# zorino/kaamer

Measured on AMD Instinct MI355X. Metric: k-mer lookups/sec, higher is better.
Workload: dtype u32

## Files before the change

kaamer_amd/csrc/count_async.hip.inc:

```

#define CA_NCTX 2u
#define CA_ARENA (GRP_BUDGET - 64u + GRP_MAX_TABLE)
#define CA_NONE 0xFFFFFFFFu
#define GRP_WQ 64u

template <bool FIRSTPOS>
__global__ __launch_bounds__(64 * GRP_WAVES, FIRSTPOS ? 5 : 6) void count_async_kernel(CountParams p)
{
    constexpr int WAVES = GRP_WAVES;
    constexpr int XIT = 2;
    constexpr bool PACKED = FIRSTPOS;
    __shared__ uint32_t a_keys[CA_ARENA];
    __shared__ uint32_t a_cnt[CA_ARENA];
    __shared__ uint32_t c_q[CA_NCTX][GRP_QMAX];
    __shared__ uint16_t c_tab[CA_NCTX][GRP_QMAX], c_cap[CA_NCTX][GRP_QMAX];
    __shared__ uint8_t c_ovf[CA_NCTX][GRP_QMAX];
    __shared__ uint32_t c_pref[CA_NCTX][GRP_QMAX + 1];
    __shared__ uint64_t c_aa[CA_NCTX][GRP_QMAX];
    __shared__ uint32_t c_hits[CA_NCTX][GRP_QMAX];
    __shared__ uint8_t c_wq[CA_NCTX][GRP_WQ];
    __shared__ uint8_t c_sq[CA_NCTX][CA_ARENA / 64];
    __shared__ uint32_t c_seq[CA_NCTX];
    __shared__ uint32_t c_nq[CA_NCTX], c_npos[CA_NCTX], c_nwin[CA_NCTX], c_tb[CA_NCTX];
    __shared__ uint32_t c_str0[CA_NCTX], c_nstr[CA_NCTX];
    __shared__ uint32_t c_need[CA_NCTX];
    __shared__ unsigned long long c_ebase[CA_NCTX];
    __shared__ uint32_t c_wdone[CA_NCTX], c_sticket[CA_NCTX], c_sdone[CA_NCTX];
    __shared__ uint32_t c_retired[CA_NCTX];
    __shared__ uint2 s_ent[CA_NCTX];
    __shared__ uint32_t s_ticket;
    __shared__ uint32_t s_built, s_tb_end, s_arena_end, s_build_lock, s_nret;
    __shared__ uint32_t s_hint;
    __shared__ uint32_t s_pref[WAVES][64];
    __shared__ uint8_t s_own[WAVES][XIT * 64];
    __shared__ unsigned long long s_tot[8];
    enum { T_IN = 0, T_Q, T_POST, T_HITS, T_OVF, T_LISTS, T_LIDS };

    const uint32_t tid = threadIdx.x, lane = tid & 63u, wv = tid >> 6;
#ifdef KAAMER_PHASE_CLOCK
    const unsigned long long ca_t0 = PHASE_T();
    unsigned long long ca_win = 0, ca_str = 0, ca_bld = 0, ca_idle = 0, ca_nwin = 0;
#define CA_CLK(acc, expr) { const unsigned long long t_ = PHASE_T(); expr; acc += PHASE_T() - t_; }
#else
#define CA_CLK(acc, expr) { expr; }
#endif
    const unsigned long long below = (1ull << lane) - 1ull;
    const uint32_t n_groups = *p.d_n_groups;
    const uint32_t nq_total = *p.d_nq;
    const uint32_t n_sched_raw = *p.d_n_sched;
    const uint32_t n_sched = n_sched_raw & 0x7FFFFFFFu;
    const bool sched_identity = (n_sched_raw >> 31) != 0u;
    const uint32_t K = n_sched > blockIdx.x ? (n_sched - 1u - blockIdx.x) / gridDim.x + 1u : 0u;
    if (K == 0u) return;

    auto ld = [&](uint32_t *w) { return __hip_atomic_load(w, __ATOMIC_RELAXED, __HIP_MEMORY_SCOPE_WORKGROUP); };
    auto st = [&](uint32_t *w, uint32_t v) { __hip_atomic_store(w, v, __ATOMIC_RELAXED, __HIP_MEMORY_SCOPE_WORKGROUP); };
    auto uni = [&](uint32_t v) { return (uint32_t)__builtin_amdgcn_readfirstlane((int)v); };
    auto sched_entry = [&](uint32_t k) {
        const uint32_t t = blockIdx.x + k * gridDim.x;
        if (k >= K) return make_uint2(0xFFFFFFFFu, GRP_NONE);
        const uint2 e = sched_identity ? make_uint2(t, p.group_first[t]) : p.sched[t];
        return make_uint2(uni(e.x), uni(e.y));
    };

    if (tid < 8) s_tot[tid] = 0;
    for (uint32_t i = tid; i < WAVES * XIT * 64; i += 64 * WAVES) (&s_own[0][0])[i] = 0;
    for (uint32_t i = tid; i < CA_ARENA; i += 64 * WAVES) {
        a_keys[i] = KH_EMPTY_PID;
        a_cnt[i] = PACKED ? 0xFFFF0000u : 0u;
    }
    if (tid == 0) {
        s_ticket = 0; s_built = 0; s_tb_end = 0; s_arena_end = 0; s_build_lock = 0; s_nret = 0; s_hint = 0;
        for (uint32_t c = 0; c < CA_NCTX; c++) { c_seq[c] = CA_NONE; c_retired[c] = 0; c_wdone[c] = 0; c_sticket[c] = 0; c_sdone[c] = 0; c_nwin[c] = 0; c_nstr[c] = 0; }
    }
    if (wv == 0) { const uint2 e = sched_entry(0u); if (lane == 0) s_ent[0] = e; }
    __syncthreads();

    auto retire = [&](uint32_t c) {
        const uint32_t nqp = c_nq[c];
        if (lane < nqp) {
            const uint32_t j = lane, q = c_q[c][j];
            if (c_ovf[c][j]) {
                atomicAdd(&s_tot[T_OVF], 1ull);
                const uint32_t slot = atomicAdd(p.ovf_count, 1u);
                WorkItem wi;
                wi.q = q; wi.size = p.qinfo[q].size; wi.aa_off = c_aa[c][j];
                if (slot < p.list_cap) p.ovf_list[slot] = wi;
                else atomicOr(p.status, (uint32_t)ST_LIST_FULL);
                p.q_cnt[q] = 0;
                p.hit_off[q] = 0;
            } else {
                const unsigned long long base = c_ebase[c] + c_tab[c][j];
                const bool have = base + c_cap[c][j] <= p.hit_cap;
                if (!have) atomicOr(p.status, (uint32_t)ST_POOL_FULL);
                p.q_cnt[q] = have ? c_hits[c][j] : 0u;
                p.hit_off[q] = have ? base : 0;
            }
        }
        __builtin_amdgcn_fence(__ATOMIC_RELEASE, "workgroup", "local");
        if (lane == 0) {
            st(&c_retired[c], ld(&c_seq[c]) + 1u);
            atomicAdd(&s_nret, 1u);
            atomicAdd(&s_hint, 1u);
        }
    };

    auto build = [&](uint32_t k) {
        const uint32_t c = k & 1u;
        if (lane == 0) st(&c_seq[c], CA_NONE);
        __builtin_amdgcn_fence(__ATOMIC_RELEASE, "workgroup", "local");
        const uint2 e = s_ent[c];
        const uint32_t gidb = e.x, firstb = e.y;
        const uint2 en = sched_entry(k + 1u);
        QInfo pre_qi;
        pre_qi.size = 0; pre_qi.slots = 0; pre_qi.aa_off = 0;
        uint64_t pre_e = 0;
        if (firstb != GRP_NONE && gidb < n_groups && (uint64_t)firstb + lane < nq_total) { pre_qi = p.qinfo[firstb + lane]; pre_e = p.slot_off[firstb + lane]; }
        const uint64_t e_first = __shfl(pre_e, 0, 64);
        uint32_t nq = 0, pos_carry = 0, slots_end = 0;
        uint64_t q0 = firstb;
        bool done = firstb == GRP_NONE || gidb >= n_groups;
        while (!done) {
            const uint64_t q = q0 + lane;
            const bool in_range = q < nq_total;
            QInfo qi;
            qi.size = 0; qi.slots = 0; qi.aa_off = 0;
            uint64_t eq = 0;
            if (q0 == firstb) { qi = pre_qi; eq = pre_e; }
            else if (in_range) { qi = p.qinfo[q]; eq = p.slot_off[q]; }
            const bool searched = in_range && qi.slots != 0;
            const bool beyond = !in_range || (searched && (eq >> GRP_SHIFT) > gidb);
            const unsigned long long bm = __ballot(beyond);
            const uint32_t cutoff = bm ? (uint32_t)__ffsll((long long)bm) - 1 : 64u;
            const bool mine = searched && lane < cutoff;
            const unsigned long long mm = __ballot(mine);
            const uint32_t szm = mine ? (uint32_t)qi.size : 0u;
            const uint32_t inc = wave_inclusive_scan_dpp(szm);
            const uint32_t tab = (uint32_t)(eq - e_first);
            if (mine) {
                const uint32_t idx = nq + (uint32_t)__popcll(mm & below);
                if (idx < GRP_QMAX) {
                    const uint32_t lo = pos_carry + inc - szm, hi = pos_carry + inc;
                    c_q[c][idx] = (uint32_t)q;
                    c_aa[c][idx] = qi.aa_off;
                    c_tab[c][idx] = (uint16_t)tab;
                    c_cap[c][idx] = (uint16_t)qi.slots;
                    c_ovf[c][idx] = (PACKED && qi.size >= 65535) ? 1u : 0u;
                    c_pref[c][idx] = lo;
                    c_hits[c][idx] = 0u;
                    for (uint32_t w = (lo + 63u) >> 6; (w << 6) < hi && w < GRP_WQ; w++) c_wq[c][w] = (uint8_t)idx;
                }
            }
            if (mm) {
                const int last = 63 - __builtin_clzll(mm);
                slots_end = (uint32_t)__builtin_amdgcn_readlane((int)(tab + qi.slots), last);
            }
            pos_carry += (uint32_t)__builtin_amdgcn_readlane((int)inc, 63);
            nq += (uint32_t)__popcll(mm);
            done = bm != 0;
            q0 += 64;
        }
        if (nq > GRP_QMAX) nq = GRP_QMAX;
        if (slots_end > CA_ARENA) slots_end = CA_ARENA;
        const uint32_t prev_end = ld(&s_arena_end);
        const uint32_t base = prev_end + slots_end <= CA_ARENA ? prev_end : 0u;
        uint32_t need = CA_NONE;
        if (k > 0u) {
            const uint32_t pc = c ^ 1u;
            const uint32_t pb = ld(&c_str0[pc]) << 6, pe = pb + (ld(&c_nstr[pc]) << 6);
            if (base < pe && pb < base + slots_end) need = k - 1u;
        }
        __builtin_amdgcn_fence(__ATOMIC_ACQ_REL, "wavefront");
        __builtin_amdgcn_wave_barrier();
        if (lane < nq) {
            const uint32_t t0 = base + c_tab[c][lane], cp = c_cap[c][lane];
            c_tab[c][lane] = (uint16_t)t0;
            for (uint32_t s = t0 >> 6; s < ((t0 + cp) >> 6) && s < CA_ARENA / 64; s++) c_sq[c][s] = (uint8_t)lane;
        }
        const uint32_t n_win = (pos_carry + 63u) >> 6;
        __builtin_amdgcn_fence(__ATOMIC_RELEASE, "workgroup", "local");
        if (lane == 0) {
            c_pref[c][nq] = pos_carry;
            c_nq[c] = nq; c_npos[c] = pos_carry; c_nwin[c] = n_win;
            c_str0[c] = base >> 6; c_nstr[c] = slots_end >> 6;
            c_need[c] = need;
            c_ebase[c] = e_first - (unsigned long long)base;
            const uint32_t tb = ld(&s_tb_end);
            c_tb[c] = tb;
            st(&s_tb_end, tb + n_win);
            st(&s_arena_end, base + slots_end);
            c_wdone[c] = 0; c_sticket[c] = 0; c_sdone[c] = 0;
            s_ent[c ^ 1u] = en;
            atomicAdd(&s_tot[T_Q], (unsigned long long)nq);
            atomicAdd(&s_tot[T_IN], (unsigned long long)pos_carry + 6ull * nq);
        }
        __builtin_amdgcn_fence(__ATOMIC_RELEASE, "workgroup", "local");
        if (lane == 0) st(&c_seq[c], k);
        if (n_win == 0u) {
            retire(c);
        }
        __builtin_amdgcn_fence(__ATOMIC_RELEASE, "workgroup", "local");
        if (lane == 0) { st(&s_built, k + 1u); st(&s_build_lock, 0u); }
    };
    auto try_build = [&]() -> bool {
        const uint32_t k = ld(&s_built);
        if (k >= K) return false;
        if (k >= CA_NCTX && ld(&c_retired[k & 1u]) != k - 1u) return false;
        uint32_t got = 0;
        if (lane == 0) got = atomicCAS(&s_build_lock, 0u, 1u) == 0u ? 1u : 0u;
        if (!uni(got)) return false;
        __builtin_amdgcn_fence(__ATOMIC_ACQUIRE, "workgroup", "local");
        if (ld(&s_built) != k) { if (lane == 0) st(&s_build_lock, 0u); return false; }
        build(k);
        return true;
    };

    auto try_stripes = [&](uint32_t c) -> bool {
        const uint32_t sq = uni(ld(&c_seq[c]));
        if (sq == CA_NONE) return false;
        const uint32_t nw = uni(ld(&c_nwin[c])), nst = uni(ld(&c_nstr[c]));
        const uint32_t wd = uni(ld(&c_wdone[c])), stk = uni(ld(&c_sticket[c]));
        __builtin_amdgcn_fence(__ATOMIC_ACQUIRE, "workgroup", "local");
        if (uni(ld(&c_seq[c])) != sq) return false;
        if (nw == 0u || wd != nw || stk >= nst) return false;
        bool did = false;
        const uint32_t s0 = uni(ld(&c_str0[c]));
        const unsigned long long ebase = c_ebase[c];
        constexpr uint32_t CA_SCH = 4;
        for (;;) {
            uint32_t t = 0;
            if (lane == 0) t = atomicAdd(&c_sticket[c], CA_SCH);
            t = uni(t);
            if (t >= nst) break;
            did = true;
            const uint32_t n_here = nst - t < CA_SCH ? nst - t : CA_SCH;
            uint32_t kk[CA_SCH], ww[CA_SCH], jj[CA_SCH];
#pragma unroll
            for (uint32_t u = 0; u < CA_SCH; u++) {
                const uint32_t s = s0 + t + (u < n_here ? u : 0u);
                const uint32_t slot = (s << 6) + lane;
                jj[u] = (uint32_t)c_sq[c][s];
                kk[u] = a_keys[slot];
                ww[u] = a_cnt[slot];
            }
            uint32_t tb_[CA_SCH], cp_[CA_SCH], ov_[CA_SCH];
#pragma unroll
            for (uint32_t u = 0; u < CA_SCH; u++) {
                jj[u] = uni(jj[u]);
                tb_[u] = c_tab[c][jj[u]]; cp_[u] = c_cap[c][jj[u]]; ov_[u] = c_ovf[c][jj[u]];
            }
#pragma unroll
            for (uint32_t u = 0; u < CA_SCH; u++) {
                if (u >= n_here) break;
                const uint32_t slot = ((s0 + t + u) << 6) + lane;
                a_keys[slot] = KH_EMPTY_PID;
                a_cnt[slot] = PACKED ? 0xFFFF0000u : 0u;
                const unsigned long long base = ebase + tb_[u];
                const bool usable = ov_[u] == 0u && base + cp_[u] <= p.hit_cap;
                const bool has = usable && kk[u] != KH_EMPTY_PID;
                const unsigned long long bm = __ballot(has);
                if (bm) {
                    uint32_t off = 0;
                    if (lane == 0) {
                        off = atomicAdd(&c_hits[c][jj[u]], (uint32_t)__popcll(bm));
                        atomicAdd(&s_tot[T_HITS], (unsigned long long)__popcll(bm));
                    }
                    off = uni(off);
                    if (has) {
                        const unsigned long long idx = base + off + (uint32_t)__popcll(bm & below);
                        p.hit_pid[idx] = kk[u];
                        p.hit_km[idx] = PACKED ? (ww[u] & 0xFFFFu) : ww[u];
                        if (FIRSTPOS) p.hit_fp[idx] = ww[u] >> 16;
                    }
                }
            }
            __builtin_amdgcn_fence(__ATOMIC_RELEASE, "workgroup", "local");
            uint32_t d = 0;
            if (lane == 0) d = atomicAdd(&c_sdone[c], n_here);
            if (uni(d) + n_here == nst) { __builtin_amdgcn_fence(__ATOMIC_ACQUIRE, "workgroup", "local"); retire(c); break; }
        }
        return did;
    };
    auto help = [&]() -> bool {
        bool did = false, d2 = false;
        CA_CLK(ca_str, did = try_stripes(0u); did = try_stripes(1u) || did);
        CA_CLK(ca_bld, d2 = try_build());
        return did || d2;
    };

    struct Job { uint32_t valid, w, c, npos, nq, need; };
    uint32_t my_k = 0;
    bool at_end = false;
    uint32_t g_tb = 0, g_nw = 0, g_c = 0, g_npos = 0, g_nq = 0, g_need = CA_NONE;
    auto try_resolve = [&](uint32_t t, Job &j) -> bool {
        for (;;) {
            if (t - g_tb < g_nw) { j.valid = 1u; j.w = t - g_tb; j.c = g_c; j.npos = g_npos; j.nq = g_nq; j.need = g_need; return true; }
            if (my_k >= K) { at_end = true; j.valid = 0u; j.w = 0u; j.c = 0u; j.npos = 0u; j.nq = 0u; j.need = CA_NONE; return true; }
            if (uni(ld(&s_built)) <= my_k) return false;
            __builtin_amdgcn_fence(__ATOMIC_ACQUIRE, "workgroup", "local");
            const uint32_t c = my_k & 1u;
            if (uni(ld(&c_seq[c])) == my_k) {
                const uint32_t tb = ld(&c_tb[c]), nw = ld(&c_nwin[c]), np = ld(&c_npos[c]), nqq = ld(&c_nq[c]), nd = ld(&c_need[c]);
                __builtin_amdgcn_fence(__ATOMIC_ACQUIRE, "workgroup", "local");
                if (uni(ld(&c_seq[c])) != my_k) continue;
                if (t - uni(tb) < uni(nw)) {
                    g_tb = uni(tb); g_nw = uni(nw); g_c = c; g_npos = uni(np); g_nq = uni(nqq); g_need = uni(nd);
                    continue;
                }
            }
            g_nw = 0u;
            my_k++;
        }
    };
    struct RawA { uint32_t vraw, j, ps; };
    auto issue_a = [&](const Job &jb) {
        RawA r;
        const uint32_t c = jb.c, w = jb.w;
        const uint32_t nqb = jb.nq, npb = jb.npos;
        const uint32_t i = (w << 6) + lane;
        const bool valid = jb.valid != 0u && i < npb;
        uint32_t j = 0;
        if (valid) {
            if (w < GRP_WQ) {
                j = c_wq[c][w];
                while (j + 1 < nqb && c_pref[c][j + 1] <= i) j++;
            } else {
#pragma unroll
                for (uint32_t sft = GRP_QMAX / 2; sft > 0; sft >>= 1)
                    if (j + sft < nqb && c_pref[c][j + sft] <= i) j += sft;
            }
        }
        r.j = j;
        r.ps = valid ? i - c_pref[c][j] : 0u;
        r.vraw = p.vals[valid ? c_aa[c][j] + r.ps : 0ull];
        return r;
    };
    auto lane_valid = [&](const Job &jb) { return jb.valid != 0u && ((jb.w << 6) + lane) < jb.npos; };
    auto issue_b = [&](uint32_t v) { return reinterpret_cast<const uint4 *>(p.arena)[(v & KH_INLINE_BIT) ? 0u : v]; };

    uint32_t c_post = 0, c_lists = 0, c_lids = 0;
    uint32_t *const pref = s_pref[wv];
    uint8_t *const own = s_own[wv];
    auto add_n = [&](uint32_t c, uint32_t j, uint32_t pid, uint32_t pos, uint32_t n) {
        const uint32_t base = c_tab[c][j], cap = c_cap[c][j];
        uint32_t hh = (uint32_t)(((uint64_t)(pid * 0x9E3779B1u) * cap) >> 32);
        const uint32_t tmax = cap < GRP_MAX_PROBES ? cap : GRP_MAX_PROBES;
        for (uint32_t t = 0; t < tmax; t++) {
            const uint32_t old = atomicCAS(&a_keys[base + hh], KH_EMPTY_PID, pid);
            const uint32_t kk = old == KH_EMPTY_PID ? pid : old;
            if (kk == pid) {
                atomicAdd(&a_cnt[base + hh], n);
                if (PACKED) {
                    uint32_t o = __hip_atomic_load(&a_cnt[base + hh], __ATOMIC_RELAXED, __HIP_MEMORY_SCOPE_WORKGROUP);
                    while (pos < (o >> 16)) {
                        const uint32_t seen = atomicCAS(&a_cnt[base + hh], o, (o & 0xFFFFu) | (pos << 16));
                        if (seen == o) break;
                        o = seen;
                    }
                }
                return;
            }
            hh = (hh + 1u == cap) ? 0u : hh + 1u;
        }
        c_ovf[c][j] = 1;
    };
    auto add_runs = [&](uint32_t c, uint32_t j, uint32_t x, uint32_t pos) {
        const uint32_t px = __shfl_up(x, 1, 64), pj = __shfl_up(j, 1, 64);
        const bool change = (lane == 0) || px != x || pj != j;
        const unsigned long long cm = __ballot(change);
        if (change && x != KH_EMPTY_PID) {
            const unsigned long long above = (lane == 63) ? 0ull : (cm >> (lane + 1));
            const uint32_t len = above ? (uint32_t)__ffsll((long long)above) : 64u - lane;
            add_n(c, j, x, pos, len);
        }
    };
    auto count_window = [&](uint32_t c, uint32_t v, uint32_t wj, uint32_t wps, const uint4 &hv) {
        const uint32_t inl = (v & KH_INLINE_BIT) ? 0xFFFFFFFFu : 0u;
        const uint32_t lcnt = hv.x | (inl & 1u), id0 = hv.y | (inl & v & ~KH_INLINE_BIT);
        if (lcnt > c_cap[c][wj] && lcnt != 0u) c_ovf[c][wj] = 1u;
        const bool dead = lcnt != 0u && c_ovf[c][wj] != 0u;
        if (lcnt != 0u) {
            c_post += lcnt;
            if (!(v & KH_INLINE_BIT)) { c_lists++; c_lids += lcnt; }
        }
        const uint32_t extra = (lcnt > 1u && !dead) ? lcnt - 1u : 0u;
        const uint32_t inc = wave_inclusive_scan_dpp(extra);
        const uint32_t xtotal = (uint32_t)__builtin_amdgcn_readlane((int)inc, 63);
        pref[lane] = inc - extra;
        if (extra != 0u && inc - extra < XIT * 64u) own[inc - extra] = (uint8_t)(lane + 1u);
        __builtin_amdgcn_fence(__ATOMIC_ACQ_REL, "wavefront");
        __builtin_amdgcn_wave_barrier();
        uint32_t carry = 0;
        uint32_t xid[XIT], xld[XIT], xm[XIT], xj[XIT], xps[XIT];
#pragma unroll
        for (int it = 0; it < XIT; it++) {
            const uint32_t t = (uint32_t)it * 64u + lane;
            const bool act = t < xtotal;
            uint32_t mk = own[t];
            own[t] = 0;
            mk = wave_inclusive_max_dpp(mk > carry ? mk : carry);
            carry = (uint32_t)__builtin_amdgcn_readlane((int)mk, 63);
            const uint32_t lo = act ? mk - 1u : 0u;
            const uint32_t off = __shfl(v, (int)lo, 64);
            const uint32_t oz = __shfl(hv.z, (int)lo, 64), ow = __shfl(hv.w, (int)lo, 64);
            xj[it] = __shfl(wj, (int)lo, 64);
            xps[it] = __shfl(wps, (int)lo, 64);
            const uint32_t k = act ? t - pref[lo] : 0u;
            const bool from_arena = act && k >= 2u;
            xld[it] = p.arena[from_arena ? (uint64_t)off * 4 + 2 + k : 0ull];
            xm[it] = from_arena ? 0xFFFFFFFFu : 0u;
            xid[it] = !act ? KH_EMPTY_PID : k == 0u ? oz : ow;
        }
        add_runs(c, wj, (lcnt > 0 && !dead) ? id0 : KH_EMPTY_PID, wps);
#pragma unroll
        for (int it = 0; it < XIT; it++) {
            const uint32_t id = (xld[it] & xm[it]) | (xid[it] & ~xm[it]);
            if (id != KH_EMPTY_PID) add_n(c, xj[it], id, xps[it], 1u);
        }
        if (xtotal > XIT * 64u) {
            for (uint32_t t0 = XIT * 64u; t0 < xtotal; t0 += GRP_LONG_UNROLL * 64u) {
                uint32_t lid[GRP_LONG_UNROLL], lj[GRP_LONG_UNROLL], lp[GRP_LONG_UNROLL];
#pragma unroll
                for (int u = 0; u < (int)GRP_LONG_UNROLL; u++) {
                    const uint32_t t = t0 + (uint32_t)u * 64u + lane;
                    const bool act = t < xtotal;
                    const uint32_t tt = act ? t : xtotal - 1u;
                    uint32_t lo = 0;
#pragma unroll
                    for (int sft = 32; sft > 0; sft >>= 1)
                        if (pref[lo + sft] <= tt) lo += sft;
                    const uint32_t off = __shfl(v, (int)lo, 64);
                    const uint32_t oz = __shfl(hv.z, (int)lo, 64), ow = __shfl(hv.w, (int)lo, 64);
                    lj[u] = __shfl(wj, (int)lo, 64);
                    lp[u] = __shfl(wps, (int)lo, 64);
                    const uint32_t k = tt - pref[lo];
                    const uint32_t ldv = p.arena[k >= 2u ? (uint64_t)off * 4 + 2 + k : 0ull];
                    const uint32_t m = k >= 2u ? 0xFFFFFFFFu : 0u;
                    const uint32_t idr = k == 0u ? oz : ow;
                    lid[u] = act ? ((ldv & m) | (idr & ~m)) : KH_EMPTY_PID;
                }
#pragma unroll
                for (int u = 0; u < (int)GRP_LONG_UNROLL; u++)
                    if (lid[u] != KH_EMPTY_PID && !c_ovf[c][lj[u]]) add_n(c, lj[u], lid[u], lp[u], 1u);
            }
        }
        __builtin_amdgcn_fence(__ATOMIC_ACQ_REL, "wavefront");
        __builtin_amdgcn_wave_barrier();
    };

    if (wv == 0) build(0u);
    __syncthreads();
    if (wv == 1 && K > 1u) {
        uint32_t got = 0;
        if (lane == 0) got = atomicCAS(&s_build_lock, 0u, 1u) == 0u ? 1u : 0u;
        if (uni(got)) build(1u);
    }

    Job j0, j1;
    j0.valid = j1.valid = 0u; j0.w = j1.w = 0u; j0.c = j1.c = 0u; j0.npos = j1.npos = 0u; j0.nq = j1.nq = 0u; j0.need = j1.need = CA_NONE;
    RawA a0, a1;
    a0.vraw = a0.j = a0.ps = 0u;
    a1 = a0;
    uint32_t v0 = 0;
    uint4 hv0 = make_uint4(0, 0, 0, 0);
    uint32_t tp = 0;
    bool have_tp = false;
    uint32_t spins = 0, seen_hint = 0xFFFFFFFFu;
    for (;;) {
        Job j2;
        j2.valid = 0u; j2.w = 0u; j2.c = 0u; j2.npos = 0u; j2.nq = 0u; j2.need = CA_NONE;
        if (!at_end) {
            if (!have_tp) {
                if (lane == 0) tp = atomicAdd(&s_ticket, 1u);
                tp = uni(tp);
                have_tp = true;
            }
            if (try_resolve(tp, j2)) have_tp = false;
            else if (!j0.valid && !j1.valid) {
                if (!help()) { CA_CLK(ca_idle, __builtin_amdgcn_s_sleep(2)); if (++spins > (1u << 24)) { if (lane == 0) atomicOr(p.status, (uint32_t)ST_CHAIN_TIMEOUT); break; } }
                continue;
            }
        }
        if (at_end && !j0.valid && !j1.valid && !j2.valid) break;
        const RawA a2 = issue_a(j2);
        const uint32_t v1 = lane_valid(j1) ? a1.vraw : 0u;
        const uint4 hv1 = issue_b(v1);
        if (j0.valid) {
            const uint32_t c = j0.c;
            const uint32_t need = j0.need;
            if (need != CA_NONE) {
                while (ld(&c_retired[need & 1u]) <= need) {
                    if (!help()) { CA_CLK(ca_idle, __builtin_amdgcn_s_sleep(1)); if (++spins > (1u << 24)) { if (lane == 0) atomicOr(p.status, (uint32_t)ST_CHAIN_TIMEOUT); break; } }
                }
                __builtin_amdgcn_fence(__ATOMIC_ACQUIRE, "workgroup", "local");
            }
            CA_CLK(ca_win, count_window(c, v0, a0.j, a0.ps, hv0));
#ifdef KAAMER_PHASE_CLOCK
            ca_nwin++;
#endif
            __builtin_amdgcn_fence(__ATOMIC_RELEASE, "workgroup", "local");
            if (lane == 0 && atomicAdd(&c_wdone[c], 1u) + 1u == (j0.npos + 63u) >> 6) atomicAdd(&s_hint, 1u);
        }
        a0 = a1; v0 = v1; hv0 = hv1; a1 = a2;
        j0 = j1; j1 = j2;
        {
            const uint32_t h = uni(ld(&s_hint));
            if (h != seen_hint) { seen_hint = h; help(); }
        }
    }
    while (ld(&s_nret) < K) {
        if (!help()) { CA_CLK(ca_idle, __builtin_amdgcn_s_sleep(2)); if (++spins > (1u << 24)) { if (lane == 0) atomicOr(p.status, (uint32_t)ST_CHAIN_TIMEOUT); break; } }
    }
    {
        const uint32_t a = wave_total(c_post), b = wave_total(c_lists), c = wave_total(c_lids);
        if (lane == 0) {
            atomicAdd(&s_tot[T_POST], (unsigned long long)a);
            atomicAdd(&s_tot[T_LISTS], (unsigned long long)b);
            atomicAdd(&s_tot[T_LIDS], (unsigned long long)c);
        }
    }
#ifdef KAAMER_PHASE_CLOCK
    if (lane == 0 && blockIdx.x < 2048) {
        unsigned long long *g = g_phase_clock[blockIdx.x];
        atomicAdd(&g[0], ca_nwin); atomicAdd(&g[1], ca_win); atomicAdd(&g[2], ca_str); atomicAdd(&g[3], ca_bld); atomicAdd(&g[4], ca_idle);
        atomicAdd(&g[5], PHASE_T() - ca_t0); atomicAdd(&g[7], 1ull);
    }
#endif
    __syncthreads();
    if (tid == 0) {
        const uint32_t rep = blockIdx.x;
        add_counter(p.counters, rep, CTR_IN, s_tot[T_IN]);
        add_counter(p.counters, rep, CTR_QUERIES, s_tot[T_Q]);
        add_counter(p.counters, rep, CTR_POST, s_tot[T_POST]);
        add_counter(p.counters, rep, CTR_HITS, s_tot[T_HITS]);
        add_counter(p.counters, rep, CTR_OVERFLOW, s_tot[T_OVF]);
        add_counter(p.counters, rep, CTR_LISTS, s_tot[T_LISTS]);
        add_counter(p.counters, rep, CTR_LIST_IDS, s_tot[T_LIDS]);
    }
}
#undef CA_CLK
```

kaamer_amd/csrc/count_group.hip.inc:

```

#ifndef GRP_WAVES
#define GRP_WAVES 8
#endif
#ifndef GRP_BUDGET
#define GRP_BUDGET 2048u
#endif
#define GRP_SHIFT 11u
static_assert((1u << GRP_SHIFT) == GRP_BUDGET, "GRP_BUDGET must be 1 << GRP_SHIFT");
#define GRP_MAX_TABLE 4096u
#define GRP_MIN_TABLE 64u
#define GRP_ARENA (GRP_BUDGET + GRP_MAX_TABLE)
#define GRP_QMAX (GRP_BUDGET / GRP_MIN_TABLE)
#define GRP_FIT (GRP_BUDGET - 64u + GRP_MAX_TABLE)
#define GRP_NONE 0xFFFFFFFFu
#define GRP_MAX_PROBES 96u
#ifndef GRP_NWIN
#define GRP_NWIN 1
#endif
#ifndef GRP_V2
#define GRP_V2 1
#endif
#ifndef GRP_LONG_UNROLL
#define GRP_LONG_UNROLL 4u
#endif
// ... 46 lines not shown
    __shared__ uint64_t s_w[LAY_THREADS / 64];
    __shared__ uint64_t s_prefix;
    const uint32_t nq = *d_nq;
    const uint64_t base = (uint64_t)blockIdx.x * LAY_TILE;
    if (base > nq) return;
    const uint32_t tid = threadIdx.x, lane = tid & 63u, wv = tid >> 6;
    uint32_t v[LAY_ITEMS];
    uint64_t sum = 0;
    const uint64_t i0 = base + (uint64_t)tid * LAY_ITEMS;
#pragma unroll
    for (int i = 0; i < LAY_ITEMS; i++) {
        v[i] = i0 + i < nq ? slots[i0 + i] : 0u;
        sum += v[i];
    }
    uint64_t inc = sum;
#pragma unroll
    for (int o = 1; o < 64; o <<= 1) {
        const uint64_t t = __shfl_up(inc, o, 64);
        if ((int)lane >= o) inc += t;
    }
    if (lane == 63) s_w[wv] = inc;
    __syncthreads();
    uint64_t woff = 0, tile_total = 0;
#pragma unroll
    for (int i = 0; i < LAY_THREADS / 64; i++) {
        if (i < (int)wv) woff += s_w[i];
        tile_total += s_w[i];
    }
    if (wv == 0) {
        unsigned long long prefix = 0;
        if (blockIdx.x > 0) {
            if (lane == 0)
                __hip_atomic_store(&chain[blockIdx.x], chain_pack(epoch, 1u, tile_total), __ATOMIC_RELAXED, __HIP_MEMORY_SCOPE_AGENT);
            long long j = (long long)blockIdx.x - 1;
            uint32_t spins = 0;
            bool done = false;
            while (!done) {
                const long long idx = j - (long long)lane;
                unsigned long long w = chain_pack(epoch, 2u, 0ull);
                if (idx >= 0) w = __hip_atomic_load(&chain[idx], __ATOMIC_RELAXED, __HIP_MEMORY_SCOPE_AGENT);
                const uint32_t flag = (uint32_t)(w >> (CHAIN_VAL_BITS + 2)) == epoch ? (uint32_t)(w >> CHAIN_VAL_BITS) & 3u : 0u;
                const unsigned long long m_inc = __ballot(flag == 2u), m_inv = __ballot(flag == 0u);
                const uint32_t first_inc = m_inc ? (uint32_t)__ffsll((long long)m_inc) - 1u : 64u;
                const unsigned long long need = first_inc >= 63u ? ~0ull : ((2ull << first_inc) - 1ull);
                if (m_inv & need) {
                    if (++spins > (1u << 20)) { if (lane == 0) atomicOr(status, (uint32_t)ST_CHAIN_TIMEOUT); break; }
                    __builtin_amdgcn_s_sleep(1);
                    continue;
                }
                unsigned long long part = lane <= first_inc ? (w & CHAIN_VAL_MASK) : 0ull;
#pragma unroll
                for (int o = 32; o > 0; o >>= 1) part += __shfl_xor(part, o, 64);
                prefix += part;
                done = first_inc < 64u;
                j -= 64;
            }
        }
        if (lane == 0) {
            __hip_atomic_store(&chain[blockIdx.x], chain_pack(epoch, 2u, prefix + tile_total), __ATOMIC_RELAXED, __HIP_MEMORY_SCOPE_AGENT);
            s_prefix = prefix;
        }
    }
    __syncthreads();
    uint64_t ex = s_prefix + woff + inc - sum;
    if (i0 == 0 && nq > 0 && groups_cap > 0) { group_first[0] = 0u; group_start[0] = 0; }
#pragma unroll
    for (int i = 0; i < LAY_ITEMS; i++) {
        const uint64_t idx = i0 + i;
        if (idx <= nq) E[idx] = ex;
        if (idx == nq) {
            uint64_t ng = ex ? ((ex - 1) >> bshift) + 1 : 0;
            if (ng > groups_cap) { atomicOr(status, (uint32_t)ST_LIST_FULL); ng = 0; }
            *d_n_groups = (uint32_t)ng;
        }
        if (idx < nq && v[i]) {
            const uint64_t g = ex >> bshift, g_hi = (ex + v[i]) >> bshift;
            for (uint64_t gg = g + 1; gg <= g_hi && gg < groups_cap; gg++) {
                group_first[gg] = gg == g_hi ? (uint32_t)(idx + 1) : GRP_NONE;
                group_start[gg] = ex + v[i];
            }
        }
        ex += v[i];
    }
}

#define SCHED_MAX_GROUPS 32768u
__global__ __launch_bounds__(1024) void schedule_kernel(const uint32_t *group_first, const uint64_t *group_start, const uint64_t *E,
                                                        const uint32_t *d_n_groups, const uint32_t *d_nq, uint2 *sched, uint32_t *d_n_sched,
                                                        uint32_t cshift)
{
    __shared__ uint32_t s_hist[16], s_base[16], s_cur[16];
    __shared__ uint8_t s_cls[SCHED_MAX_GROUPS];
    const uint32_t ng = *d_n_groups, tid = threadIdx.x;
    if (ng > SCHED_MAX_GROUPS) {
        if (tid == 0) *d_n_sched = ng | 0x80000000u;
        return;
    }
    const uint64_t total = E[*d_nq];
    if (tid < 16) { s_hist[tid] = 0; s_cur[tid] = 0; }
    __syncthreads();
    for (uint32_t g = tid; g < ng; g += 1024) {
        uint32_t c = 0xFFu;
        if (group_first[g] != GRP_NONE) {
            const uint64_t ext = (g + 1 < ng ? group_start[g + 1] : total) - group_start[g];
            c = (uint32_t)(ext >> cshift);
            c = c > 15u ? 15u : c;
            atomicAdd(&s_hist[c], 1u);
        }
        s_cls[g] = (uint8_t)c;
    }
    __syncthreads();
    if (tid == 0) {
        uint32_t run = 0;
        for (int c = 15; c >= 0; c--) { s_base[c] = run; run += s_hist[c]; }
        *d_n_sched = run;
    }
    __syncthreads();
    for (uint32_t g = tid; g < ng; g += 1024) {
        const uint32_t c = s_cls[g];
        if (c != 0xFFu) sched[s_base[c] + atomicAdd(&s_cur[c], 1u)] = make_uint2(g, group_first[g]);
    }
}

struct PrepLayoutParams {
    const uint8_t *seqs;
    const uint64_t *offsets;
    uint32_t n_seqs;
    uint64_t pos_bound;
    kaamer_query_meta *q;
    uint32_t *d_nq;
    unsigned long long *d_n_pos;
    unsigned long long *invalid;
    QInfo *qinfo;
    uint64_t *hit_off;
    uint32_t *q_cnt;
    uint64_t *E;
    uint32_t *group_first;
    uint64_t *group_start;
    uint32_t *d_n_groups;
    uint32_t groups_cap;
    unsigned long long *chain;
    uint32_t epoch;
    uint32_t *status;
    uint2 *sched;
    uint32_t *d_n_sched;
    uint32_t *slots;
    uint32_t bshift;
    uint32_t cshift;
    uint32_t no_sched;
    uint32_t *tiles_done;
    unsigned long long *d_total;
    const uint32_t *slot_scale;
    unsigned long long room_slots;
};

#define PL_ITEMS 1
#define PL_TILE (LAY_THREADS * PL_ITEMS)
__global__ __launch_bounds__(LAY_THREADS) void prep_layout_schedule_kernel(PrepLayoutParams p)
{
    __shared__ uint64_t s_w[LAY_THREADS / 64];
    __shared__ uint64_t s_prefix;
    __shared__ uint32_t s_slots[PL_TILE];
    __shared__ uint32_t s_last;
    const uint32_t nq = p.n_seqs;
    const uint64_t base = (uint64_t)blockIdx.x * PL_TILE;
    const uint32_t tid = threadIdx.x, lane = tid & 63u, wv = tid >> 6;
    const bool batch_bad = p.offsets[nq] > p.pos_bound;
    const uint32_t slot_scale = p.slot_scale ? fit_table_scale(*p.slot_scale, batch_bad ? 0ull : p.offsets[nq], nq, p.room_slots) : SLOT_SCALE_ONE;
    if (blockIdx.x == 0 && tid == 0) {
        const uint64_t n_pos = batch_bad ? 0 : p.offsets[nq];
        if (batch_bad) atomicOr(p.status, (uint32_t)ST_AA_CAP);
        *p.d_nq = nq;
        *p.d_n_pos = n_pos;
        mark_invalid_range(p.invalid, n_pos, (n_pos + 63) & ~63ull);
    }
#pragma unroll
    for (int r = 0; r < PL_ITEMS; r++) {
        const uint64_t i = base + (uint64_t)r * LAY_THREADS + tid;
        uint32_t slots = 0;
        if (i < nq) {
            uint64_t b = p.offsets[i], e = p.offsets[i + 1];
            if (batch_bad || e < b || e > p.pos_bound) {
                if (!batch_bad) atomicOr(p.status, (uint32_t)ST_AA_CAP);
                b = e = 0;
            }
            const int64_t len = (int64_t)(e - b);
            int32_t size = (int32_t)(len - KAAMER_KMER_SIZE + 1);
            if (len > 0 && p.seqs[e - 1] == '*') size--;
            kaamer_query_meta m;
            m.src_seq = (uint32_t)i;
            m.size_in_kmer = size;
            m.start_position = 1;
            m.end_position = (int32_t)len;
            m.plus_strand = 1;
            m.aa_len = (uint32_t)len;
            m.aa_off = b;
            m.sa_off = 0;
            m.sa_len = 0;
            p.q[i] = m;
            p.q_cnt[i] = 0;
            p.hit_off[i] = 0;
            QInfo qi;
            qi.size = size;
            qi.aa_off = b;
            if (size >= 7) {
                qi.slots = table_slots_for(size, slot_scale);
                mark_invalid_range(p.invalid, b + (uint64_t)size, e);
            } else {
                qi.slots = 0;
                mark_invalid_range(p.invalid, b, e);
            }
            p.qinfo[i] = qi;
            p.slots[i] = qi.slots;
            slots = qi.slots;
        }
        s_slots[r * LAY_THREADS + tid] = slots;
    }
    __syncthreads();
    uint32_t v[PL_ITEMS];
    uint64_t sum = 0;
    const uint64_t i0 = base + (uint64_t)tid * PL_ITEMS;
#pragma unroll
    for (int i = 0; i < PL_ITEMS; i++) {
        v[i] = s_slots[tid * PL_ITEMS + i];
        sum += v[i];
    }
    uint64_t inc = sum;
#pragma unroll
    for (int o = 1; o < 64; o <<= 1) {
        const uint64_t t = __shfl_up(inc, o, 64);
        if ((int)lane >= o) inc += t;
    }
    if (lane == 63) s_w[wv] = inc;
    __syncthreads();
    uint64_t woff = 0, tile_total = 0;
#pragma unroll
    for (int i = 0; i < LAY_THREADS / 64; i++) {
        if (i < (int)wv) woff += s_w[i];
        tile_total += s_w[i];
    }
    if (wv == 0) {
        unsigned long long prefix = 0;
        if (blockIdx.x > 0) {
            if (lane == 0)
                __hip_atomic_store(&p.chain[blockIdx.x], chain_pack(p.epoch, 1u, tile_total), __ATOMIC_RELAXED, __HIP_MEMORY_SCOPE_AGENT);
            long long j = (long long)blockIdx.x - 1;
            uint32_t spins = 0;
            bool done = false;
            while (!done) {
                const long long idx = j - (long long)lane;
                unsigned long long w = chain_pack(p.epoch, 2u, 0ull);
                if (idx >= 0) w = __hip_atomic_load(&p.chain[idx], __ATOMIC_RELAXED, __HIP_MEMORY_SCOPE_AGENT);
                const uint32_t flag = (uint32_t)(w >> (CHAIN_VAL_BITS + 2)) == p.epoch ? (uint32_t)(w >> CHAIN_VAL_BITS) & 3u : 0u;
                const unsigned long long m_inc = __ballot(flag == 2u), m_inv = __ballot(flag == 0u);
                const uint32_t first_inc = m_inc ? (uint32_t)__ffsll((long long)m_inc) - 1u : 64u;
                const unsigned long long need = first_inc >= 63u ? ~0ull : ((2ull << first_inc) - 1ull);
                if (m_inv & need) {
                    if (++spins > (1u << 20)) { if (lane == 0) atomicOr(p.status, (uint32_t)ST_CHAIN_TIMEOUT); break; }
                    __builtin_amdgcn_s_sleep(1);
                    continue;
                }
                unsigned long long part = lane <= first_inc ? (w & CHAIN_VAL_MASK) : 0ull;
#pragma unroll
                for (int o = 32; o > 0; o >>= 1) part += __shfl_xor(part, o, 64);
                prefix += part;
                done = first_inc < 64u;
                j -= 64;
            }
        }
        if (lane == 0) {
            __hip_atomic_store(&p.chain[blockIdx.x], chain_pack(p.epoch, 2u, prefix + tile_total), __ATOMIC_RELAXED, __HIP_MEMORY_SCOPE_AGENT);
            s_prefix = prefix;
        }
    }
    __syncthreads();
    uint64_t ex = s_prefix + woff + inc - sum;
    if (i0 == 0 && nq > 0 && p.groups_cap > 0) {
        __hip_atomic_store(&p.group_first[0], 0u, __ATOMIC_RELAXED, __HIP_MEMORY_SCOPE_AGENT);
        __hip_atomic_store(&p.group_start[0], (uint64_t)0, __ATOMIC_RELAXED, __HIP_MEMORY_SCOPE_AGENT);
    }
#pragma unroll
    for (int i = 0; i < PL_ITEMS; i++) {
        const uint64_t idx = i0 + i;
        if (idx <= nq) p.E[idx] = ex;
        if (idx == nq) {
            uint64_t ng = ex ? ((ex - 1) >> p.bshift) + 1 : 0;
            if (ng > p.groups_cap) { atomicOr(p.status, (uint32_t)ST_LIST_FULL); ng = 0; }
            __hip_atomic_store(p.d_n_groups, (uint32_t)ng, __ATOMIC_RELAXED, __HIP_MEMORY_SCOPE_AGENT);
            __hip_atomic_store(p.d_total, (unsigned long long)ex, __ATOMIC_RELAXED, __HIP_MEMORY_SCOPE_AGENT);
            if (p.no_sched) *p.d_n_sched = (uint32_t)ng | 0x80000000u;
        }
        if (idx < nq && v[i]) {
            const uint64_t g = ex >> p.bshift, g_hi = (ex + v[i]) >> p.bshift;
            for (uint64_t gg = g + 1; gg <= g_hi && gg < p.groups_cap; gg++) {
                __hip_atomic_store(&p.group_first[gg], gg == g_hi ? (uint32_t)(idx + 1) : GRP_NONE, __ATOMIC_RELAXED, __HIP_MEMORY_SCOPE_AGENT);
                __hip_atomic_store(&p.group_start[gg], (uint64_t)(ex + v[i]), __ATOMIC_RELAXED, __HIP_MEMORY_SCOPE_AGENT);
            }
        }
        ex += v[i];
    }
    if (p.no_sched) return;
    asm volatile("s_waitcnt vmcnt(0) lgkmcnt(0)" ::: "memory");
    __syncthreads();
    if (tid == 0) s_last = atomicAdd(p.tiles_done, 1u) == gridDim.x - 1u;
    __syncthreads();
    if (!s_last) return;
    if (tid == 0) __hip_atomic_store(p.tiles_done, 0u, __ATOMIC_RELAXED, __HIP_MEMORY_SCOPE_AGENT);
    uint32_t *s_hist = s_slots, *s_base = s_slots + 16, *s_cur = s_slots + 32;
    __shared__ uint8_t s_cls[SCHED_MAX_GROUPS];
    const uint32_t ng = __hip_atomic_load(p.d_n_groups, __ATOMIC_RELAXED, __HIP_MEMORY_SCOPE_AGENT);
    if (ng > SCHED_MAX_GROUPS) {
        if (tid == 0) *p.d_n_sched = ng | 0x80000000u;
        return;
    }
    const uint64_t total = __hip_atomic_load(p.d_total, __ATOMIC_RELAXED, __HIP_MEMORY_SCOPE_AGENT);
    if (tid < 16) { s_hist[tid] = 0; s_cur[tid] = 0; }
    __syncthreads();
    for (uint32_t g = tid; g < ng; g += LAY_THREADS) {
        uint32_t c = 0xFFu;
        if (__hip_atomic_load(&p.group_first[g], __ATOMIC_RELAXED, __HIP_MEMORY_SCOPE_AGENT) != GRP_NONE) {
            const uint64_t nxt = g + 1 < ng ? __hip_atomic_load(&p.group_start[g + 1], __ATOMIC_RELAXED, __HIP_MEMORY_SCOPE_AGENT) : total;
            const uint64_t ext = nxt - __hip_atomic_load(&p.group_start[g], __ATOMIC_RELAXED, __HIP_MEMORY_SCOPE_AGENT);
            c = (uint32_t)(ext >> p.cshift);
            c = c > 15u ? 15u : c;
            atomicAdd(&s_hist[c], 1u);
        }
        s_cls[g] = (uint8_t)c;
    }
    __syncthreads();
    if (tid == 0) {
        uint32_t run = 0;
        for (int c = 15; c >= 0; c--) { s_base[c] = run; run += s_hist[c]; }
        *p.d_n_sched = run;
    }
    __syncthreads();
    for (uint32_t g = tid; g < ng; g += LAY_THREADS) {
        const uint32_t c = s_cls[g];
        if (c != 0xFFu)
            p.sched[s_base[c] + atomicAdd(&s_cur[c], 1u)] =
                make_uint2(g, __hip_atomic_load(&p.group_first[g], __ATOMIC_RELAXED, __HIP_MEMORY_SCOPE_AGENT));
    }
}

__device__ __forceinline__ uint32_t wave_inclusive_scan_dpp(uint32_t v)
{
#define KH_DPP_ADD(ctrl, rmask) v += (uint32_t)__builtin_amdgcn_update_dpp(0, (int)v, ctrl, rmask, 0xf, false)
    KH_DPP_ADD(0x111, 0xf);
    KH_DPP_ADD(0x112, 0xf);
    KH_DPP_ADD(0x114, 0xf);
    KH_DPP_ADD(0x118, 0xf);
    KH_DPP_ADD(0x142, 0xa);
    KH_DPP_ADD(0x143, 0xc);
#undef KH_DPP_ADD
    return v;
}

__device__ __forceinline__ uint32_t wave_inclusive_max_dpp(uint32_t v)
{
#define KH_DPP_MAX(ctrl, rmask) { const uint32_t t_ = (uint32_t)__builtin_amdgcn_update_dpp(0, (int)v, ctrl, rmask, 0xf, false); v = v > t_ ? v : t_; }
    KH_DPP_MAX(0x111, 0xf);
    KH_DPP_MAX(0x112, 0xf);
    KH_DPP_MAX(0x114, 0xf);
    KH_DPP_MAX(0x118, 0xf);
// ... 820 lines not shown
```

kaamer_amd/csrc/search.hip:

```cpp
#include <hip/hip_runtime.h>

#include <dlfcn.h>

#include <algorithm>
#include <cstdarg>
#include <cstdio>
#include <cstdlib>
#include <cstring>
#include <condition_variable>
#include <memory>
#include <mutex>
#include <new>
#include <vector>

#include "kaamer_internal.h"

static thread_local char g_err[512] = "";

int kaamer_fail(int code, const char *fmt, ...)
{
    va_list ap;
    va_start(ap, fmt);
    vsnprintf(g_err, sizeof g_err, fmt, ap);
    va_end(ap);
    return code;
}

#define HIPCHK(expr)                                                                          \
    do {                                                                                      \
        hipError_t e_ = (expr);                                                               \
        if (e_ != hipSuccess)                                                                 \
            return kaamer_fail(KAAMER_E_HIP, "%s failed: %s", #expr, hipGetErrorString(e_)); \
    } while (0)

struct kaamer_workspace;
struct HostSlot {
    kaamer_workspace *ws = nullptr;
    kaamer_workspace_opts opts{};
    uint8_t *d_seqs = nullptr;
    uint64_t *d_off = nullptr;
    size_t seq_cap = 0, off_cap = 0;
    hipStream_t stream = nullptr;
    bool busy = false;
};

struct TopSlot {
    kaamer_workspace *ws = nullptr;
    kaamer_workspace_opts opts{};
    hipStream_t stream = nullptr;
    uint8_t *d_seqs = nullptr;
    uint64_t *d_off = nullptr;
    size_t seq_cap = 0, off_cap = 0;
    uint8_t *h_in = nullptr;
    size_t h_in_cap = 0;
    uint8_t *d_block = nullptr;
    size_t d_block_cap = 0;
    size_t guess = 1u << 16;
    bool busy = false;
};
#define KAAMER_MAX_HOST_SLOTS 8
static void top_slot_free(TopSlot &h);

struct kaamer_index {
    int device;
    kh_image_header hdr;
    kh_bucket *d_buckets;
    uint32_t *d_arena;
    HostSlot host[4];
    std::mutex pool_mu;
    std::condition_variable pool_cv;
    TopSlot top[KAAMER_MAX_HOST_SLOTS];
    int n_top;
};

enum { ST_POOL_FULL = 1u, ST_LIST_FULL = 2u, ST_QUERY_CAP = 4u, ST_AA_CAP = 8u, ST_G_ARENA_FULL = 16u, ST_G_TABLE_FULL = 32u,
       ST_POS_UNSUPPORTED = 64u, ST_POS_CAP = 128u, ST_CHAIN_TIMEOUT = 256u, ST_EXCHANGE_CAP = 512u, ST_PEER_FAILED = 1024u };
enum { CTR_IN = 0, CTR_QUERIES, CTR_LOOKUP, CTR_PROBE, CTR_FOUND, CTR_POST, CTR_HITS, CTR_OVERFLOW, CTR_LISTS, CTR_LIST_IDS, CTR_N };
static_assert(sizeof(kaamer_counters) == CTR_N * 8, "counter layout");
#define CTR_REPLICAS 64

enum { LIST_S = 0, LIST_L, LIST_SO, LIST_G, N_LISTS };
enum { SLOT_QUEUE_HEAD = N_LISTS, SLOT_STATUS = N_LISTS + 1, SLOT_GROUP_QUEUE = N_LISTS + 2, SLOT_GROUP_QUEUE_POS = N_LISTS + 3,
       SLOT_N_LONG = N_LISTS + 4, SLOT_TILES_DONE = N_LISTS + 5, SLOT_TR_TICKET = N_LISTS + 6,
       SLOT_QUEUE_SUB = N_LISTS + 7 , SLOT_G_TICKET = N_LISTS + 15, SLOT_PACK_TICKETS = N_LISTS + 16 ,
       SLOT_G_HITS16 = N_LISTS + 80 ,
       SLOT_G_MON_HITS16 = N_LISTS + 81 , SLOT_G_MONSTERS = N_LISTS + 82 ,
       N_SMALL_SLOTS = N_LISTS + 16 + 64 + 3 };
#define G_MONSTER_HITS (GRP_MAX_TABLE / 4u * 3u)
static_assert(N_SMALL_SLOTS <= 256, "the finalize step zeroes one slot per thread");
struct alignas(16) WorkItem {
    uint32_t q;
    int32_t size;
    uint64_t aa_off;
};

#define CURSOR_STRIDE 32u
#define MAX_TIMED_CALLS 1024u
#define L_WAVES 8
#define L_LOG2CAP 12
#define G_WAVES 8
#ifndef S_MIN_WAVES
#define S_MIN_WAVES 1
#endif
#ifndef L_MIN_WAVES
#define L_MIN_WAVES 1
#endif
#ifndef S_NWIN
#define S_NWIN 3
#endif

__device__ __forceinline__ uint32_t lane_id() { return threadIdx.x & 63u; }

__device__ __forceinline__ uint32_t wave_sum32(uint32_t v)
{
#pragma unroll
    for (int o = 32; o > 0; o >>= 1) v += __shfl_xor(v, o, 64);
    return v;
}
__device__ __forceinline__ uint32_t wave_total(uint32_t v)
{
    return (uint32_t)__builtin_amdgcn_readfirstlane((int)wave_sum32(v));
}

__device__ __forceinline__ void add_counter(unsigned long long *replicas, uint32_t replica, int which, unsigned long long v)
{
    if (v) atomicAdd(&replicas[(size_t)(replica % CTR_REPLICAS) * CTR_N + which], v);
}

struct ProbeParams {
    const uint4 *table;
    uint64_t n_buckets;
    uint32_t n_shards, shard;
    const uint8_t *residues;
    unsigned long long *invalid;
    const unsigned long long *d_n_pos;
    uint32_t *vals;
    unsigned long long *counters;
    uint32_t nontemporal;
};

#define P_WAVES 4
#define P_RING 128u
#define KH_NO_KEY 0xFFFFFFFDu

template <bool SKIP_IDLE> __global__ __launch_bounds__(64 * P_WAVES) void probe_kernel(ProbeParams p)
{
    __shared__ uint8_t s_lut[256];
    __shared__ uint8_t s_stage[P_WAVES][80];
    __shared__ uint32_t s_ring[P_WAVES][3][P_RING];
    const uint32_t tid = threadIdx.x, lane = tid & 63u;
    const uint32_t wv = (uint32_t)__builtin_amdgcn_readfirstlane((int)(tid >> 6));
    const unsigned long long n_pos = *p.d_n_pos;
    const unsigned long long n_win = (n_pos + 63) >> 6;
    for (uint32_t i = tid; i < 256; i += 64 * P_WAVES) s_lut[i] = (uint8_t)kh_residue_code((uint8_t)i);
    __syncthreads();
    uint32_t c_lookup = 0, c_probe = 0, c_found = 0;
    uint8_t *stage = s_stage[wv];
    uint32_t *const ring_key = s_ring[wv][0], *const ring_pos = s_ring[wv][1], *const ring_step = s_ring[wv][2];
    uint32_t ring_head = 0, ring_n = 0;
    const uint32_t n_buckets = (uint32_t)p.n_buckets;
    const uint32_t mine = 16u * (lane & 3u) + (lane >> 2);

    const unsigned long long stride = (unsigned long long)gridDim.x * P_WAVES;
    unsigned long long w = (unsigned long long)blockIdx.x * P_WAVES + wv;
    unsigned long long mask = 0;
    uint32_t ra = 0, rb = 0;
    auto fetch = [&](unsigned long long win, unsigned long long &m, uint32_t &a, uint32_t &b) {
        const unsigned long long wc = win < n_win ? win : n_win - 1;
        m = p.invalid[wc];
        const unsigned long long i0 = (wc << 6) + lane, last = n_pos - 1;
        a = p.residues[i0 < last ? i0 : last];
        b = p.residues[i0 + 64 < last ? i0 + 64 : last];
    };
    if (n_win) fetch(w, mask, ra, rb);

    while (n_win) {
        const bool ring = ring_n >= 64u || (w >= n_win && ring_n > 0u);
        if (!ring && w >= n_win) break;
        unsigned long long base = 0;
        uint32_t key = KH_NO_KEY, off = lane, step = 0;
        if (ring) {
            const uint32_t n = ring_n < 64u ? ring_n : 64u;
            if (lane < n) {
                const uint32_t slot = (ring_head + lane) & (P_RING - 1u);
                key = ring_key[slot]; off = ring_pos[slot]; step = ring_step[slot];
            }
            ring_head = (ring_head + n) & (P_RING - 1u);
            ring_n -= n;
        } else {
            base = w << 6;
            stage[lane] = s_lut[ra];
            if (lane < 6) stage[64 + lane] = s_lut[rb];
            __builtin_amdgcn_fence(__ATOMIC_ACQ_REL, "wavefront");
            __builtin_amdgcn_wave_barrier();
            const uint8_t *st = stage + lane;
            key = kh_key_from_codes(st[0], st[1], st[2], st[3], st[4], st[5], st[6]);
            const bool own = p.n_shards <= 1 || kh_shard_of(key, p.n_shards) == p.shard;
            key = (((~mask >> lane) & 1ull) && own) ? key : KH_NO_KEY;
            __builtin_amdgcn_fence(__ATOMIC_ACQ_REL, "wavefront");
            __builtin_amdgcn_wave_barrier();
            c_lookup += key != KH_NO_KEY ? 1u : 0u;
        }
        c_probe += key != KH_NO_KEY ? 1u : 0u;
        const unsigned long long w_cur = w;
        if (!ring) w += stride;
        fetch(w, mask, ra, rb);

        uint32_t my_bucket = 0u;
        if (key != KH_NO_KEY) {
            my_bucket = (uint32_t)kh_home_bucket(key, p.n_shards, p.n_buckets) + step;
            my_bucket = my_bucket >= n_buckets ? my_bucket - n_buckets : my_bucket;
        }
        uint4 ld[4];
        uint32_t rk[4];
#pragma unroll
        for (int j = 0; j < 4; j++) {
            const int src = 16 * j + (int)(lane >> 2);
            rk[j] = __shfl(key, src, 64);
            const uint32_t bucket = __shfl(my_bucket, src, 64);
            typedef uint32_t v4u __attribute__((ext_vector_type(4)));
            const v4u *srcp = reinterpret_cast<const v4u *>(p.table) + (uint64_t)bucket * 4 + (lane & 3u);
            if (SKIP_IDLE) {
                ld[j] = make_uint4(KH_EMPTY_KEY, 0u, KH_EMPTY_KEY, 0u);
                if (rk[j] != KH_NO_KEY) {
                    const v4u t = *srcp;
                    ld[j] = make_uint4(t.x, t.y, t.z, t.w);
                }
            } else {
                const v4u t = p.nontemporal ? __builtin_nontemporal_load(srcp) : *srcp;
                ld[j] = make_uint4(t.x, t.y, t.z, t.w);
            }
        }
        uint32_t okey = KH_NO_KEY, oval = 0, oempty = 1u;
#pragma unroll
        for (int j = 0; j < 4; j++) {
            const uint32_t kk = rk[j];
            uint32_t r = (ld[j].x == kk) ? ld[j].y : ((ld[j].z == kk) ? ld[j].w : 0u);
            uint32_t e = (ld[j].x == KH_EMPTY_KEY || ld[j].z == KH_EMPTY_KEY) ? 1u : 0u;
            r |= (uint32_t)__builtin_amdgcn_update_dpp(0, (int)r, 0xB1, 0xf, 0xf, false);
            e |= (uint32_t)__builtin_amdgcn_update_dpp(0, (int)e, 0xB1, 0xf, 0xf, false);
            r |= (uint32_t)__builtin_amdgcn_update_dpp(0, (int)r, 0x4E, 0xf, 0xf, false);
            e |= (uint32_t)__builtin_amdgcn_update_dpp(0, (int)e, 0x4E, 0xf, 0xf, false);
            const bool take = (lane & 3u) == (uint32_t)j;
            okey = take ? kk : okey; oval = take ? r : oval; oempty = take ? e : oempty;
        }
        const uint32_t ooff = __shfl(off, (int)mine, 64);
        const bool valid = okey != KH_NO_KEY;
        c_found += (valid && oval != 0u) ? 1u : 0u;
        const unsigned long long W = __ballot(valid && oval == 0u && oempty == 0u);
        if (W) {
            const uint32_t ostep = __shfl(step, (int)mine, 64);
            const bool wk = valid && oval == 0u && oempty == 0u && ostep + 1u < n_buckets;
            const unsigned long long W2 = __ballot(wk);
            if (wk) {
                const uint32_t slot = (ring_head + ring_n + (uint32_t)__builtin_amdgcn_mbcnt_hi((uint32_t)(W2 >> 32), __builtin_amdgcn_mbcnt_lo((uint32_t)W2, 0u))) & (P_RING - 1u);
                ring_key[slot] = okey;
                ring_pos[slot] = (uint32_t)base + ooff;
                ring_step[slot] = ostep + 1u;
            }
            ring_n += (uint32_t)__popcll(W2);
        }
        __builtin_amdgcn_fence(__ATOMIC_ACQ_REL, "wavefront");
        __builtin_amdgcn_wave_barrier();
        if (!ring || oval != 0u) p.vals[base + ooff] = oval;
        if (lane == 0) p.invalid[ring ? n_win + 1 : w_cur] = 0ull;
    }
    const uint32_t t_lookup = wave_total(c_lookup), t_probe = wave_total(c_probe), t_found = wave_total(c_found);
    if (lane == 0) {
        const uint32_t rep = blockIdx.x * P_WAVES + wv;
        add_counter(p.counters, rep, CTR_LOOKUP, t_lookup);
        add_counter(p.counters, rep, CTR_PROBE, t_probe);
        add_counter(p.counters, rep, CTR_FOUND, t_found);
    }
}

struct QInfo;
struct CountParams {
    const uint32_t *arena;
    const uint32_t *vals;
    const struct QInfo *qinfo;
    const uint64_t *slot_off;
    uint32_t *group_first;
    const uint32_t *d_n_groups;
    const uint32_t *d_nq;
    uint32_t last_group_pass;
    uint32_t pack_shift;
    uint32_t *pack_tickets;
    const uint64_t *pos_base;
    unsigned long long *pos_bits;
    const uint32_t *m_pid, *m_km, *m_fp;
    uint32_t merge_fp;
    const WorkItem *list;
    const uint32_t *list_count;
    WorkItem *ovf_list;
    uint32_t *ovf_count;
    uint32_t list_cap;
    uint32_t *queue_head;
    uint32_t *group_queue;
    const uint2 *sched;
    const uint32_t *d_n_sched;
    uint64_t *hit_off;
    uint32_t *q_cnt;
    uint32_t *hit_pid, *hit_km, *hit_fp;
    uint64_t hit_cap;
    unsigned long long *tail_cursor;
    uint32_t *g_keys;
    uint64_t g_slots;
    unsigned long long *g_cursor;
    uint32_t n_proteins;
    unsigned long long *counters;
    uint32_t *status;
    kaamer_counters *fin_out;
    uint32_t *fin_small, *fin_status_out;
    unsigned long long *fin_cursors;
    uint32_t *fin_slot_scale;
    uint32_t fin_scale_cap, fin_scale_margin;
};

__device__ __forceinline__ unsigned long long tail_alloc(const CountParams &p, uint32_t total)
{
    const unsigned long long b = p.slot_off[*p.d_nq] + atomicAdd(p.tail_cursor, (unsigned long long)total);
    if (b + total > p.hit_cap) { atomicOr(p.status, (uint32_t)ST_POOL_FULL); return ~0ull; }
    return b;
}

template <int LOG2CAP, bool FIRSTPOS = true> struct LdsTable {
    volatile uint32_t *keys;
    uint32_t *cnt, *minpos, *nd;
    static constexpr uint32_t CAP = 1u << LOG2CAP;
    static constexpr uint32_t LIMIT = CAP - CAP / 4;
    __device__ __forceinline__ bool add_n(uint32_t pid, uint32_t pos, uint32_t n, uint32_t &nnew) const
    {
        constexpr uint32_t MASK = CAP - 1u;
        uint32_t h = (pid * 0x9E3779B1u) >> (32 - LOG2CAP);
        for (uint32_t t = 0; t <= MASK; t++) {
            uint32_t k = keys[h];
            if (k == KH_EMPTY_PID) {
                const uint32_t old = atomicCAS((uint32_t *)&keys[h], KH_EMPTY_PID, pid);
                if (old == KH_EMPTY_PID) { nnew++; k = pid; }
                else k = old;
            }
            if (k == pid) {
                atomicAdd(&cnt[h], n);
                if (FIRSTPOS) atomicMin(&minpos[h], pos);
                return true;
            }
            h = (h + 1u) & MASK;
        }
        return false;
    }
    __device__ __forceinline__ bool over_limit() const { return *(volatile uint32_t *)nd > LIMIT; }
};

#define BIG_LOG2CAP 13
struct BigLdsTable {
    uint32_t *keys, *val, *nd;
    static constexpr uint32_t CAP = 1u << BIG_LOG2CAP;
    static constexpr uint32_t LIMIT = CAP - CAP / 4;
    __device__ __forceinline__ bool add_n(uint32_t pid, uint32_t pos, uint32_t n, uint32_t &nnew) const
    {
        uint32_t h = (pid * 0x9E3779B1u) >> (32 - BIG_LOG2CAP);
        for (uint32_t t = 0; t < 128u; t++) {
            uint32_t k = __hip_atomic_load(&keys[h], __ATOMIC_RELAXED, __HIP_MEMORY_SCOPE_WORKGROUP);
            if (k == KH_EMPTY_PID) {
                const uint32_t old = atomicCAS(&keys[h], KH_EMPTY_PID, pid);
                if (old == KH_EMPTY_PID) { k = pid; if (atomicAdd(nd, 1u) >= LIMIT) return false; }
                else k = old;
            }
            if (k == pid) {
                atomicAdd(&val[h], n);
                uint32_t old = __hip_atomic_load(&val[h], __ATOMIC_RELAXED, __HIP_MEMORY_SCOPE_WORKGROUP);
                while (pos < (old >> 16)) {
                    const uint32_t seen = atomicCAS(&val[h], old, (old & 0xFFFFu) | (pos << 16));
                    if (seen == old) break;
                    old = seen;
                }
                return true;
            }
            h = (h + 1u) & (CAP - 1u);
        }
        return false;
    }
    __device__ __forceinline__ bool over_limit() const { return false; }
};

#define G_MAX_RANGES 64u
__device__ __forceinline__ uint32_t g_range_of(uint32_t pid, uint32_t R) { return (uint32_t)(((uint64_t)(pid * 0x85EBCA6Bu) * R) >> 32); }
struct RangeHist {
    uint32_t *cnt, *nd;
    uint32_t R;
    __device__ __forceinline__ bool add_n(uint32_t pid, uint32_t, uint32_t, uint32_t &) const { atomicAdd(&cnt[g_range_of(pid, R)], 1u); return true; }
    __device__ __forceinline__ bool over_limit() const { return false; }
};
struct RangeScatter {
    uint32_t *cur, *nd;
    uint2 *items;
    uint32_t R;
    const uint32_t *first;
    uint32_t cap;
    uint32_t *ovf;
    __device__ __forceinline__ bool add_n(uint32_t pid, uint32_t pos, uint32_t n, uint32_t &) const
    {
        const uint32_t r = g_range_of(pid, R);
        const uint32_t at = atomicAdd(&cur[r], 1u);
        if (at - first[r] < cap) items[at] = make_uint2(pid, pos | (n << 16));
        else *ovf = 1u;
        return true;
    }
    __device__ __forceinline__ bool over_limit() const { return false; }
};

struct GlobalTable {
    uint32_t *slots;
    uint32_t *nd;
    uint32_t log2cap;
    __device__ __forceinline__ bool add_n(uint32_t pid, uint32_t pos, uint32_t n, uint32_t &nnew) const
    {
        const uint32_t mask = (1u << log2cap) - 1u;
        uint32_t h = (pid * 0x9E3779B1u) >> (32 - log2cap);
        for (uint32_t t = 0; t <= mask; t++) {
            uint32_t *sl = slots + 4ull * h;
            uint32_t k = KH_EMPTY_PID;
            if (__hip_atomic_compare_exchange_strong(&sl[0], &k, pid, __ATOMIC_RELAXED, __ATOMIC_RELAXED, __HIP_MEMORY_SCOPE_WORKGROUP)) {
                nnew++;
                k = pid;
            }
            if (k == pid) {
                __hip_atomic_fetch_add(&sl[1], n, __ATOMIC_RELAXED, __HIP_MEMORY_SCOPE_WORKGROUP);
                __hip_atomic_fetch_min(&sl[2], pos, __ATOMIC_RELAXED, __HIP_MEMORY_SCOPE_WORKGROUP);
                return true;
            }
            h = (h + 1u) & mask;
// ... 85 lines not shown
#pragma unroll
        for (int k = 0; k < NWIN; k++) {
            const volatile uint32_t *pref = s_pref + k * 64;
#pragma unroll
            for (int it = 0; it < XIT; it++) {
                const uint32_t t = (uint32_t)it * 64u + lane;
                const bool act = t < xtotal[k];
                uint32_t lo = 0;
                if (act) {
#pragma unroll
                    for (int sft = 32; sft > 0; sft >>= 1)
                        if (pref[lo + sft] <= t) lo += sft;
                }
                const uint32_t off = __shfl(v[k], (int)lo, 64);
                xid[k][it] = KH_EMPTY_PID;
                xpos[k][it] = (uint32_t)(c0 + k * stride) + lo;
                if (act) xid[k][it] = p.arena[(uint64_t)off * 4 + 4 + (t - pref[lo])];
            }
        }
#pragma unroll
        for (int k = 0; k < NWIN; k++) {
            const volatile uint32_t *pref = s_pref + k * 64;
            for (uint32_t t0 = XIT * 64u; t0 < xtotal[k]; t0 += 64) {
                const uint32_t t = t0 + lane;
                const bool act = t < xtotal[k];
                uint32_t lo = 0;
                if (act) {
#pragma unroll
                    for (int sft = 32; sft > 0; sft >>= 1)
                        if (pref[lo + sft] <= t) lo += sft;
                }
                const uint32_t off = __shfl(v[k], (int)lo, 64);
                if (act) ok = ok && tab.add_n(p.arena[(uint64_t)off * 4 + 4 + (t - pref[lo])], (uint32_t)(c0 + k * stride) + lo, 1u, nnew);
            }
        }
        __builtin_amdgcn_fence(__ATOMIC_ACQUIRE, "wavefront");
        __builtin_amdgcn_wave_barrier();
    }
#pragma unroll
    for (int k = 0; k < NWIN; k++) {
        const uint32_t pos = (uint32_t)(c0 + k * stride) + lane;
        const uint32_t lcnt = h[k].x;
        if (lcnt != 0u) {
            c.post += lcnt;
            if (!(v[k] & KH_INLINE_BIT)) { c.lists++; c.lids += lcnt; }
        }
        if (!COUNT_ONLY) {
            ok = add_runs(tab, lcnt > 0 ? h[k].y : KH_EMPTY_PID, pos, nnew) && ok;
            ok = add_runs(tab, lcnt > 1 ? h[k].z : KH_EMPTY_PID, pos, nnew) && ok;
            ok = add_runs(tab, lcnt > 2 ? h[k].w : KH_EMPTY_PID, pos, nnew) && ok;
        }
    }
    if (!COUNT_ONLY) {
#pragma unroll
        for (int k = 0; k < NWIN; k++)
#pragma unroll
            for (int it = 0; it < XIT; it++)
                if (xid[k][it] != KH_EMPTY_PID) ok = ok && tab.add_n(xid[k][it], xpos[k][it], 1u, nnew);
        const uint32_t wave_new = wave_total(nnew);
        if (lane == 0 && wave_new) atomicAdd(tab.nd, wave_new);
    }
    return __all(ok);
}

__device__ __forceinline__ void mark_invalid_range(unsigned long long *invalid, uint64_t b, uint64_t e)
{
    while (b < e) {
        const uint64_t w = b >> 6;
        const uint64_t hi = ((w + 1) << 6) < e ? ((w + 1) << 6) : e;
        const unsigned nb = (unsigned)(hi - b);
        const unsigned long long m = (nb == 64 ? ~0ull : ((1ull << nb) - 1ull)) << (b & 63);
        atomicOr(&invalid[w], m);
        b = hi;
    }
}

#include "count_group.hip.inc"
#include "count_async.hip.inc"
#define PK_ARENA_PROT 1600u
#ifndef PK_ARENA_ORF
#define PK_ARENA_ORF 640u
#endif
#define PK_ARENA_ORF_LONG 1024u
#include "count_pack.hip.inc"

struct NullTable {
    uint32_t *nd;
    __device__ __forceinline__ bool add_n(uint32_t, uint32_t, uint32_t, uint32_t &) const { return true; }
    __device__ __forceinline__ bool over_limit() const { return false; }
};

template <bool IN_FLIGHT>
__device__ __forceinline__ void finalize_body(unsigned long long *replicas, kaamer_counters *out, uint32_t *small_state,
                                              uint32_t *status_out, unsigned long long *cursors, uint32_t *slot_scale = nullptr,
                                              uint32_t scale_cap = 16u, uint32_t margin_q4 = 30u)
{
    static_assert(CTR_REPLICAS == 64, "one replica per lane");
    const uint32_t lane = threadIdx.x & 63u, wv = threadIdx.x >> 6;
    for (uint32_t c = wv; c < CTR_N; c += blockDim.x >> 6) {
        unsigned long long *w = &replicas[(size_t)lane * CTR_N + c];
        unsigned long long s = IN_FLIGHT ? __hip_atomic_load(w, __ATOMIC_RELAXED, __HIP_MEMORY_SCOPE_AGENT) : *w;
        *w = 0;
#pragma unroll
        for (int o = 32; o > 0; o >>= 1) s += __shfl_xor(s, o, 64);
        if (lane == 0) ((unsigned long long *)out)[c] = s;
    }
    unsigned long long g_hits = 0, g_mon_hits = 0, g_monsters = 0;
    if (threadIdx.x == 0) {
        *status_out = IN_FLIGHT ? __hip_atomic_load(&small_state[SLOT_STATUS], __ATOMIC_RELAXED, __HIP_MEMORY_SCOPE_AGENT) : small_state[SLOT_STATUS];
        g_hits = 16ull * (IN_FLIGHT ? __hip_atomic_load(&small_state[SLOT_G_HITS16], __ATOMIC_RELAXED, __HIP_MEMORY_SCOPE_AGENT) : small_state[SLOT_G_HITS16]);
        g_mon_hits = 16ull * (IN_FLIGHT ? __hip_atomic_load(&small_state[SLOT_G_MON_HITS16], __ATOMIC_RELAXED, __HIP_MEMORY_SCOPE_AGENT) : small_state[SLOT_G_MON_HITS16]);
        g_monsters = IN_FLIGHT ? __hip_atomic_load(&small_state[SLOT_G_MONSTERS], __ATOMIC_RELAXED, __HIP_MEMORY_SCOPE_AGENT) : small_state[SLOT_G_MONSTERS];
    }
    __syncthreads();
    if (threadIdx.x < N_SMALL_SLOTS) small_state[threadIdx.x] = 0;
    if (threadIdx.x < 3) cursors[threadIdx.x * CURSOR_STRIDE] = 0;
    if (slot_scale && threadIdx.x == 0) {
        const unsigned long long nq = out->n_queries;
        const unsigned long long n_ovf = out->n_overflow < nq ? out->n_overflow : nq;
        const unsigned long long n_mon = g_monsters < n_ovf ? g_monsters : n_ovf;
        const bool widen = 8ull * (n_ovf - n_mon) > nq;
        const unsigned long long ovf = widen ? n_mon : n_ovf;
        const unsigned long long left_out = widen ? g_mon_hits : g_hits;
        const unsigned long long hits = out->n_hits > left_out ? out->n_hits - left_out : 0ull;
        const unsigned long long lookups = nq ? out->n_lookup / nq * (nq - ovf) + out->n_lookup % nq * (nq - ovf) / nq : 0ull;
        if (lookups) {
            unsigned long long t = (hits * margin_q4 + lookups - 1ull) / lookups;
            if (t < 24ull) t = 16ull;
            if (t > scale_cap) t = scale_cap;
            *slot_scale = (uint32_t)t;
        }
    }
}

#ifndef G_MIN_BLOCKS
#define G_MIN_BLOCKS 1
#endif
#ifndef G_NWIN
#define G_NWIN 2
#endif
#ifdef KAAMER_PHASE_CLOCK
__device__ unsigned long long g_gtier_clock[2048][16];
#endif
__global__ __launch_bounds__(64 * G_WAVES, G_MIN_BLOCKS) void count_global_kernel(CountParams p)
{
    constexpr int WAVES = G_WAVES;
    __shared__ uint32_t s_nd, s_fail, s_cursor;
    constexpr int NWIN = G_NWIN;
    __shared__ uint32_t s_pref[WAVES][NWIN * 64];
    __shared__ unsigned long long s_post, s_off, s_base, s_reserved;
    __shared__ uint32_t s_roff[G_MAX_RANGES], s_rcur[G_MAX_RANGES], s_rtotal;
    __shared__ LongSink s_long;
    __shared__ uint32_t b_keys[BigLdsTable::CAP], b_val[BigLdsTable::CAP];

    const uint32_t tid = threadIdx.x, lane = tid & 63u, wv = tid >> 6;
    const uint32_t n_items = *p.list_count < p.list_cap ? *p.list_count : p.list_cap;
    const uint32_t n_part = n_items < gridDim.x ? (n_items ? n_items : 1u) : gridDim.x;
    if (blockIdx.x >= n_part) return;
    unsigned long long tot_hits = 0, f_post = 0, f_lists = 0, f_lids = 0, mon_hits = 0;
    uint32_t mon_q = 0;
#ifdef KAAMER_PHASE_CLOCK
    unsigned long long gq_acc[10] = {0, 0, 0, 0, 0, 0, 0, 0, 0, 0};
    const unsigned long long gq_start = wall_clock64();
#endif
    PostCtr pc;
    NullTable nt;
    nt.nd = &s_nd;
    auto expand_long = [&](const auto &tab) {
        const uint32_t nl = s_long.n < LONG_SINK_CAP ? s_long.n : LONG_SINK_CAP;
        if (wv == 0 && nl) {
            constexpr uint32_t PER = LONG_SINK_CAP / 64;
            uint32_t sum = 0;
            for (uint32_t i = 0; i < PER; i++) { const uint32_t e = lane * PER + i; sum += e < nl ? s_long.cnt[e] : 0u; }
            uint32_t inc = sum;
#pragma unroll
            for (int o = 1; o < 64; o <<= 1) {
                const uint32_t t = __shfl_up(inc, o, 64);
                if ((int)lane >= o) inc += t;
            }
            uint32_t run = inc - sum;
            for (uint32_t i = 0; i < PER; i++) {
                const uint32_t e = lane * PER + i;
                if (e < nl) { const uint32_t c = s_long.cnt[e]; s_long.cnt[e] = run; run += c; }
            }
            if (lane == 63) s_long.total = inc;
        }
        __syncthreads();
        uint32_t nnew = 0;
        bool ok = true;
        const uint32_t total = nl ? s_long.total : 0u;
#ifndef G_EXPAND_UNROLL
#define G_EXPAND_UNROLL 8
#endif
        constexpr int EU = G_EXPAND_UNROLL;
        uint32_t e = 0;
        auto find_list = [&](uint32_t t) {
            if (e + 1u < nl && s_long.cnt[e + 1u] <= t) {
                e++;
                if (e + 1u < nl && s_long.cnt[e + 1u] <= t) {
                    e = 0;
#pragma unroll
                    for (uint32_t sft = LONG_SINK_LIFT; sft > 0; sft >>= 1)
                        if (e + sft < nl && s_long.cnt[e + sft] <= t) e += sft;
                }
            }
        };
        for (uint32_t t0 = tid; t0 < total; t0 += EU * 64 * WAVES) {
            if (s_fail) break;
            uint32_t ids[EU], pos_[EU];
#pragma unroll
            for (int u = 0; u < EU; u++) {
                const uint32_t t = t0 + (uint32_t)u * 64 * WAVES;
                const uint32_t tt = t < total ? t : total - 1u;
                find_list(tt);
                ids[u] = p.arena[(uint64_t)s_long.off[e] * 4 + 1 + (tt - s_long.cnt[e])];
                pos_[u] = s_long.pos[e];
            }
#pragma unroll
            for (int u = 0; u < EU; u++)
                if (t0 + (uint32_t)u * 64 * WAVES < total)
                    if (!tab.add_n(ids[u], pos_[u], 1u, nnew)) { ok = false; s_fail = 1; }
        }
        const uint32_t wn = wave_total(nnew);
        if (lane == 0 && wn) atomicAdd(&s_nd, wn);
        if (!ok) s_fail = 1;
    };

    __shared__ uint32_t s_item;
    for (uint32_t item = blockIdx.x; item < n_items;) {
        const WorkItem wi = p.list[item];
        const uint32_t q = wi.q;
        const bool fresh = wi.size < 0;
        const int32_t size = fresh ? -wi.size : wi.size;
        const uint32_t *vals = p.vals + wi.aa_off;
        if (tid == 0) {
            s_nd = 0; s_fail = 0; s_post = 0; s_cursor = 0; s_long.n = 0;
            s_item = atomicAdd(p.queue_head + (SLOT_G_TICKET - SLOT_QUEUE_HEAD), 1u) + n_part;
        }
        __syncthreads();
        item = s_item;
#ifdef KAAMER_PHASE_CLOCK
        unsigned long long gq_t = wall_clock64();
        const unsigned long long gq_t0 = gq_t;
#define GQ_LAP(i) { if (tid == 0) { const unsigned long long t_ = wall_clock64(); gq_acc[i] += t_ - gq_t; gq_t = t_; } }
#else
#define GQ_LAP(i) { }
#endif
        pc.clear();
        for (int32_t r0 = 0; r0 < size; r0 += 64 * WAVES * NWIN)
            count_windows<NullTable, NWIN, true>(p, vals, size, r0 + 64 * (int32_t)wv, 64 * WAVES, nt, pc, s_pref[wv]);
        {
            const unsigned long long wp = wave_total(pc.post);
            if (lane == 0 && wp) atomicAdd(&s_post, wp);
            if (fresh) {
                const uint32_t wl = wave_total(pc.lists), wi_ = wave_total(pc.lids);
                if (lane == 0) { f_post += wp; f_lists += wl; f_lids += wi_; }
            }
        }
        __syncthreads();
        if (size < 65535) {
            BigLdsTable bt;
            bt.keys = b_keys; bt.val = b_val; bt.nd = &s_nd;
            bool q_done = false, give_up = false;
            uint32_t written = 0;
            if (tid == 0) s_base = ~0ull;
            auto count_bucket = [&](uint32_t R, uint32_t r, const uint2 *items) -> int {
                __syncthreads();
                if (tid == 0) { s_nd = 0; s_fail = 0; s_cursor = 0; s_long.n = 0; }
                for (uint32_t i = tid; i < BigLdsTable::CAP; i += 64 * WAVES) { b_keys[i] = KH_EMPTY_PID; b_val[i] = 0xFFFF0000u; }
                __syncthreads();
                if (R == 1u) {
                    pc.clear();
                    for (int32_t r0 = 0; r0 < size && !s_fail; r0 += 64 * WAVES * NWIN) {
                        const bool ok = count_windows<BigLdsTable, NWIN, false>(p, vals, size, r0 + 64 * (int32_t)wv, 64 * WAVES, bt, pc,
                                                                               s_pref[wv], &s_long);
                        if (!ok) s_fail = 1;
                    }
                    __syncthreads();
                    expand_long(bt);
                } else {
                    uint32_t nnew = 0;
                    const uint32_t b0 = s_roff[r], b1 = s_rcur[r];
                    for (uint32_t i = b0 + tid; i < b1; i += 64 * WAVES) {
                        if (s_fail) break;
                        const uint2 it = items[i];
                        if (!bt.add_n(it.x, it.y & 0xFFFFu, it.y >> 16, nnew)) s_fail = 1;
                    }
                }
                __syncthreads();
                const uint32_t total = s_nd;
                if (s_fail != 0u || total > BigLdsTable::LIMIT) return 1;
                if (s_base == ~0ull && total > 0) {
                    __syncthreads();
                    if (tid == 0) {
                        unsigned long long want = total;
                        if (R > 1u) want = s_post < p.n_proteins ? s_post : p.n_proteins;
                        s_base = tail_alloc(p, (uint32_t)(want > 0xFFFFFFF0ull ? 0xFFFFFFF0ull : want));
                        s_reserved = want;
                        if (s_base == ~0ull) s_fail = 2;
                    }
                    __syncthreads();
                    if (s_fail == 2u) return 2;
                }
                const unsigned long long base = s_base;
                if (total > 0) {
                    if ((unsigned long long)written + total > s_reserved) { if (tid == 0) atomicOr(p.status, (uint32_t)ST_POOL_FULL); return 2; }
                    for (uint32_t i0 = wv * 64u; i0 < BigLdsTable::CAP; i0 += 64 * WAVES) {
                        const uint32_t k = b_keys[i0 + lane];
                        const bool has = k != KH_EMPTY_PID;
                        const unsigned long long bm = __ballot(has);
                        uint32_t wbase = 0;
                        if (lane == 0 && bm) wbase = atomicAdd(&s_cursor, (uint32_t)__popcll(bm));
                        wbase = __shfl(wbase, 0, 64);
                        if (has) {
                            const unsigned long long idx = base + written + wbase + (uint32_t)__popcll(bm & ((1ull << lane) - 1ull));
                            const uint32_t v = b_val[i0 + lane];
                            p.hit_pid[idx] = k;
                            p.hit_km[idx] = v & 0xFFFFu;
                            p.hit_fp[idx] = v >> 16;
                        }
                    }
                    written += total;
                }
                return 0;
            };
            GQ_LAP(0);
            int rc1 = count_bucket(1u, 0u, nullptr);
            GQ_LAP(1);
            if (rc1 == 0 || rc1 == 2) q_done = true;
            if (rc1 == 1) {
                uint32_t R = (uint32_t)(s_post / 16384ull) + 2u;
                if (R > G_MAX_RANGES) R = G_MAX_RANGES;
                for (int attempt = 0; attempt < 2 && !q_done; attempt++) {
                    uint32_t cap_items = 0xFFFFFFFFu;
                    __syncthreads();
                    if (tid == 0) { s_fail = 0; s_long.n = 0; s_cursor = 0; }
                    if (attempt == 0) {
                        const unsigned long long per = s_post / R;
                        const unsigned long long c = per + per / 4ull + 2048ull;
                        if (c * R > 0x7FFFFFFFull) continue;
                        cap_items = (uint32_t)c;
                        if (tid < G_MAX_RANGES) { s_roff[tid] = tid * cap_items; s_rcur[tid] = tid * cap_items; }
                        if (tid == 0) s_rtotal = R * cap_items;
                        __syncthreads();
                    } else {
                        if (tid < G_MAX_RANGES) s_roff[tid] = 0;
                        __syncthreads();
                        RangeHist rh;
                        rh.cnt = s_roff; rh.nd = &s_nd; rh.R = R;
                        pc.clear();
                        for (int32_t r0 = 0; r0 < size; r0 += 64 * WAVES * NWIN)
                            count_windows<RangeHist, NWIN, false>(p, vals, size, r0 + 64 * (int32_t)wv, 64 * WAVES, rh, pc, s_pref[wv], &s_long);
                        __syncthreads();
                        expand_long(rh);
                        __syncthreads();
                        if (wv == 0) {
                            const uint32_t v = lane < R ? s_roff[lane] : 0u;
                            uint32_t inc = v;
#pragma unroll
                            for (int o = 1; o < 64; o <<= 1) {
                                const uint32_t t = __shfl_up(inc, o, 64);
                                if ((int)lane >= o) inc += t;
                            }
                            s_roff[lane] = inc - v;
                            s_rcur[lane] = inc - v;
                            if (lane == 63) s_rtotal = inc;
                        }
                        __syncthreads();
                    }
                    const uint32_t n_items = s_rtotal;
                    if (tid == 0) {
                        const unsigned long long need = ((unsigned long long)n_items + 1ull) / 2ull + 1ull;
                        const unsigned long long off = atomicAdd(p.g_cursor, need);
                        if (off + need > p.g_slots) { atomicOr(p.status, (uint32_t)ST_G_ARENA_FULL); s_off = ~0ull; }
                        else s_off = off;
                        s_long.n = 0;
                    }
                    __syncthreads();
                    if (s_off == ~0ull) { give_up = true; q_done = true; break; }
                    uint2 *items = reinterpret_cast<uint2 *>(p.g_keys + 4ull * s_off);
                    RangeScatter rsc;
                    rsc.cur = s_rcur; rsc.items = items; rsc.nd = &s_nd; rsc.R = R;
                    rsc.first = s_roff; rsc.cap = cap_items; rsc.ovf = &s_cursor;
                    pc.clear();
                    for (int32_t r0 = 0; r0 < size; r0 += 64 * WAVES * NWIN)
                        count_windows<RangeScatter, NWIN, false>(p, vals, size, r0 + 64 * (int32_t)wv, 64 * WAVES, rsc, pc, s_pref[wv], &s_long);
                    __syncthreads();
                    expand_long(rsc);
                    __syncthreads();
                    GQ_LAP(2);
                    if (s_cursor != 0u) continue;
                    bool overflow = false;
                    for (uint32_t r = 0; r < R && !q_done; r++) {
                        const int rc = count_bucket(R, r, items);
                        if (rc == 1) { overflow = true; break; }
                        if (rc == 2) { q_done = true; give_up = true; }
                    }
                    GQ_LAP(3);
#ifdef KAAMER_PHASE_CLOCK
                    if (tid == 0) { gq_acc[6] += 1; gq_acc[7] += s_post; }
// ... 210 lines not shown
#include "translate.hip.inc"
#include "topn.hip.inc"

#define SCAN_BLOCK 1024
#define SCAN_ITEMS 16
#define SCAN_TILE (SCAN_BLOCK * SCAN_ITEMS)

__device__ __forceinline__ uint64_t block_exclusive_scan(uint64_t v, uint64_t *total)
{
    __shared__ uint64_t s_w[SCAN_BLOCK / 64];
    const uint32_t lane = threadIdx.x & 63, w = threadIdx.x >> 6;
    uint64_t inc = v;
#pragma unroll
    for (int o = 1; o < 64; o <<= 1) {
        uint64_t t = __shfl_up(inc, o, 64);
        if ((int)lane >= o) inc += t;
    }
    __syncthreads();
    if (lane == 63) s_w[w] = inc;
    __syncthreads();
    uint64_t woff = 0, tot = 0;
#pragma unroll
    for (int i = 0; i < SCAN_BLOCK / 64; i++) {
        if (i < (int)w) woff += s_w[i];
        tot += s_w[i];
    }
    *total = tot;
    return woff + inc - v;
}

__global__ __launch_bounds__(SCAN_BLOCK) void scan_single_kernel(const uint32_t *cnt, const uint32_t *d_nq, uint64_t *hit_off)
{
    const uint32_t nq = *d_nq;
    uint64_t carry = 0;
    for (uint64_t base = 0; base <= nq; base += SCAN_TILE) {
        uint32_t v[SCAN_ITEMS];
        uint64_t s = 0;
#pragma unroll
        for (int i = 0; i < SCAN_ITEMS; i++) {
            const uint64_t idx = base + (uint64_t)threadIdx.x * SCAN_ITEMS + i;
            v[i] = idx < nq ? cnt[idx] : 0u;
            s += v[i];
        }
        uint64_t tot;
        uint64_t ex = block_exclusive_scan(s, &tot) + carry;
#pragma unroll
        for (int i = 0; i < SCAN_ITEMS; i++) {
            const uint64_t idx = base + (uint64_t)threadIdx.x * SCAN_ITEMS + i;
            if (idx <= nq) hit_off[idx] = ex;
            ex += v[i];
        }
        carry += tot;
        __syncthreads();
    }
}

__global__ __launch_bounds__(SCAN_BLOCK) void scan_block_sums_kernel(const uint32_t *cnt, const uint32_t *d_nq,
                                                                    uint64_t *bsum)
{
    const uint32_t nq = *d_nq;
    const uint64_t base = (uint64_t)blockIdx.x * SCAN_TILE;
    if (base > nq) { if (threadIdx.x == 0) bsum[blockIdx.x] = 0; return; }
    uint64_t s = 0;
#pragma unroll
    for (int i = 0; i < SCAN_ITEMS; i++) {
        const uint64_t idx = base + (uint64_t)threadIdx.x * SCAN_ITEMS + i;
        if (idx < nq) s += cnt[idx];
    }
    uint64_t tot;
    block_exclusive_scan(s, &tot);
    if (threadIdx.x == 0) bsum[blockIdx.x] = tot;
}

__global__ __launch_bounds__(SCAN_BLOCK) void scan_top_kernel(uint64_t *bsum, uint32_t n_blocks)
{
    uint64_t carry = 0;
    for (uint32_t b0 = 0; b0 < n_blocks; b0 += SCAN_BLOCK) {
        const uint32_t i = b0 + threadIdx.x;
        const uint64_t v = i < n_blocks ? bsum[i] : 0;
        uint64_t tot;
        const uint64_t ex = block_exclusive_scan(v, &tot);
        if (i < n_blocks) bsum[i] = carry + ex;
        carry += tot;
        __syncthreads();
    }
}

__global__ __launch_bounds__(SCAN_BLOCK) void scan_apply_kernel(const uint32_t *cnt, const uint32_t *d_nq,
                                                               const uint64_t *bsum, uint64_t *hit_off)
{
    const uint32_t nq = *d_nq;
    const uint64_t base = (uint64_t)blockIdx.x * SCAN_TILE;
    if (base > nq) return;
    uint32_t v[SCAN_ITEMS];
    uint64_t s = 0;
#pragma unroll
    for (int i = 0; i < SCAN_ITEMS; i++) {
        const uint64_t idx = base + (uint64_t)threadIdx.x * SCAN_ITEMS + i;
        v[i] = idx < nq ? cnt[idx] : 0u;
        s += v[i];
    }
    uint64_t tot;
    uint64_t ex = block_exclusive_scan(s, &tot) + bsum[blockIdx.x];
#pragma unroll
    for (int i = 0; i < SCAN_ITEMS; i++) {
        const uint64_t idx = base + (uint64_t)threadIdx.x * SCAN_ITEMS + i;
        if (idx <= nq) hit_off[idx] = ex;
        ex += v[i];
    }
}

#include "exchange.hip.inc"

__global__ __launch_bounds__(256) void gather_hits_kernel(const uint32_t *d_nq, const uint64_t *csr_off, const uint64_t *hit_off,
                                                          const uint32_t *q_cnt, const uint32_t *in_pid, const uint32_t *in_km,
                                                          const uint32_t *in_fp, uint32_t *out_pid, uint32_t *out_km,
                                                          uint32_t *out_fp, uint64_t out_cap, uint32_t *status, int firstpos)
{
    const uint32_t nq = *d_nq;
    const uint64_t n_hits = csr_off[nq];
    if (n_hits > out_cap) { if (blockIdx.x == 0 && threadIdx.x == 0) atomicOr(status, (uint32_t)ST_POOL_FULL); return; }
    const uint32_t lane = threadIdx.x & 63u;
    const uint64_t wave = ((uint64_t)blockIdx.x * blockDim.x + threadIdx.x) >> 6;
    const uint64_t n_waves = ((uint64_t)gridDim.x * blockDim.x) >> 6;
    for (uint64_t q = wave; q < nq; q += n_waves) {
        const uint32_t n = q_cnt[q];
        if (n == 0) continue;
        const uint64_t s = hit_off[q], d = csr_off[q];
        for (uint32_t i = lane; i < n; i += 64) {
            out_pid[d + i] = in_pid[s + i];
            out_km[d + i] = in_km[s + i];
            if (firstpos) out_fp[d + i] = in_fp[s + i];
        }
    }
}

__global__ void finalize_kernel(unsigned long long *replicas, kaamer_counters *out, uint32_t *small_state,
                                uint32_t *status_out, unsigned long long *cursors, uint32_t *slot_scale, uint32_t scale_cap, uint32_t margin_q4)
{
    finalize_body<false>(replicas, out, small_state, status_out, cursors, slot_scale, scale_cap, margin_q4);
}

struct kaamer_workspace {
    int device;
    kaamer_workspace_opts opts;
    uint32_t q_cap;
    uint64_t hit_cap, sparse_cap, g_slots, pos_cap;
    bool compact;
    uint64_t *d_csr_off;
    uint32_t *d_c_pid, *d_c_km, *d_c_fp;
    int g_grid, p_grid, n_cu, pack_grid, pack_grid_long;
    bool use_group;
    bool count_async;
    int unit_windows;
    uint32_t pack_shift;
    kaamer_query_meta *d_q;
    uint32_t *d_nq;
    unsigned long long *d_n_pos;
    unsigned long long *d_valid;
    uint32_t *d_vals;
    uint32_t *d_q_cnt;
    unsigned long long *d_pool_cursor;
    WorkItem *d_lists;
    QInfo *d_qinfo;
    uint32_t *d_slots;
    uint64_t *d_slot_off;
    uint32_t *d_group_first;
    uint32_t *d_n_groups;
    uint32_t groups_cap;
    hipStream_t count_stream;
    hipEvent_t ev_probe, ev_count;
    bool split_pending;
    int grp_grid;
    bool sched_identity;
    bool nucleotide;
    uint64_t aa_cap, sa_cap;
    uint32_t *d_cnt3;
    uint64_t *d_off3;
    uint32_t *d_n6;
    uint32_t max_long;
    uint64_t max_piece_items;
    uint32_t *d_long_seq, *d_long_np, *d_pcnt3, *d_n_piece_items, *d_piece_li;
    uint64_t *d_piece_base, *d_poff3;
    kaamer_query_meta *d_tmp_meta;
    uint8_t *d_orf_aa;
    int32_t *d_starts_alt;
    uint32_t max_seqs;
    unsigned long long *d_chain;
    uint2 *d_sched;
    uint64_t *d_group_start;
    unsigned long long *d_lay_total;
    uint32_t *d_slot_scale;
    uint32_t slot_scale_cap;
    unsigned long long table_room;
    uint32_t slot_scale_margin;
    bool dense_tables;
    uint32_t *d_n_sched;
    uint32_t topn_k;
    uint32_t *d_top_cnt, *d_top_pid, *d_top_km, *d_top_fp;
    int32_t *d_top_trim, *d_top_start, *d_top_size;
    bool last_was_merge;
    size_t x_dst_cap, x_src_cap, x_ent_cap, x_m_cap;
    unsigned long long *d_x_stats;
    unsigned long long *h_x_stats;
    hipEvent_t ev_x_stats[2];
    uint64_t x_merge_seq;
    uint32_t *d_x_dst_off, *d_x_src_off, *d_x_nq_owned, *d_x_pid, *d_x_km, *d_x_fp;
    uint64_t *d_x_ent_off;
    uint64_t *d_x_tiles;
    size_t x_tiles_cap;
    size_t x_dstb_cap, x_pq_cap, x_pb_cap, x_pbits_cap;
    uint64_t *d_x_dst_boff, *d_x_src_boff, *d_x_ent_boff, *d_x_mdst;
    int32_t *d_x_msize;
    unsigned long long *d_x_mbits, *d_x_gtab;
    unsigned long long *d_x_pstats;
    uint32_t rep_k;
    uint32_t *d_rep_flag, *d_rep_aalen, *d_rep_query, *d_rep_pid, *d_rep_km, *d_rep_fp;
    int32_t *d_rep_trim;
    uint64_t *d_rep_rank, *d_rep_eoff, *d_rep_aoff, *d_rep_off;
    kaamer_query_meta *d_rep_q;
    uint8_t *d_rep_aa;
    uint32_t lay_epoch;
    unsigned long long *d_tr_chain;
    uint32_t tr_epoch;
    uint32_t *d_list_counts;
    uint32_t *d_status_out;
    bool clean;
    bool firstpos;
    bool want_positions;
    uint64_t bits_cap;
    uint32_t *d_pos_words;
    uint64_t *d_pos_base;
    uint64_t *d_pos_off;
    unsigned long long *d_pos_bits;
    uint32_t *d_g_keys;
    unsigned long long *d_counter_replicas;
    kaamer_counters *d_counters;
    uint64_t *d_bsum;
    uint32_t n_scan_blocks;
    uint64_t *d_hit_off;
    uint32_t *d_hit_pid, *d_hit_km, *d_hit_fp;
    std::vector<hipEvent_t> *ev;
    uint32_t n_timed, time_every, call_no;
};
#define EV_PER_CALL 5

template <class T> static int dev_alloc(T **p, size_t n)
{
    *p = nullptr;
    hipError_t e = hipMalloc((void **)p, (n ? n : 1) * sizeof(T));
    if (e != hipSuccess) return kaamer_fail(KAAMER_E_NOMEM, "hipMalloc(%zu bytes): %s", n * sizeof(T), hipGetErrorString(e));
    return KAAMER_OK;
}

static void launch_group(const CountParams &p, int grid, bool firstpos, hipStream_t s, bool async, int unit_windows)
{
    if (!async && unit_windows == 4) {
        if (firstpos) hipLaunchKernelGGL((count_group_kernel<true, 0, 4>), dim3(grid), dim3(64 * GRP_WAVES), 0, s, p);
        else hipLaunchKernelGGL((count_group_kernel<false, 0, 4>), dim3(grid), dim3(64 * GRP_WAVES), 0, s, p);
        return;
    }
    if (async) {
        if (firstpos) hipLaunchKernelGGL((count_async_kernel<true>), dim3(grid), dim3(64 * GRP_WAVES), 0, s, p);
        else hipLaunchKernelGGL((count_async_kernel<false>), dim3(grid), dim3(64 * GRP_WAVES), 0, s, p);
        return;
    }
    if (firstpos) hipLaunchKernelGGL((count_group_kernel<true, 0>), dim3(grid), dim3(64 * GRP_WAVES), 0, s, p);
    else hipLaunchKernelGGL((count_group_kernel<false, 0>), dim3(grid), dim3(64 * GRP_WAVES), 0, s, p);
}
static void launch_group_positions(const CountParams &p, int grid, hipStream_t s)
{
    hipLaunchKernelGGL((count_group_kernel<false, 1>), dim3(grid), dim3(64 * GRP_WAVES), 0, s, p);
}
static void launch_group_merge(const CountParams &p, int grid, bool firstpos, hipStream_t s)
{
    if (firstpos) hipLaunchKernelGGL((count_group_kernel<true, 2>), dim3(grid), dim3(64 * GRP_WAVES), 0, s, p);
    else hipLaunchKernelGGL((count_group_kernel<false, 2>), dim3(grid), dim3(64 * GRP_WAVES), 0, s, p);
}

extern "C" {

const char *kaamer_last_error(void) { return g_err; }
int kaamer_abi_version(void) { return KAAMER_ABI_VERSION; }

#ifdef KAAMER_PHASE_CLOCK
int kaamer_debug_gtier_clock(unsigned long long *out, int reset)
{
    HIPCHK(hipDeviceSynchronize());
    static unsigned long long all[2048][16];
    HIPCHK(hipMemcpyFromSymbol(all, HIP_SYMBOL(g_gtier_clock), sizeof all));
    memcpy(out, all, sizeof all);
    if (reset) { memset(all, 0, sizeof all); HIPCHK(hipMemcpyToSymbol(HIP_SYMBOL(g_gtier_clock), all, sizeof all)); }
    return KAAMER_OK;
}
int kaamer_debug_phase_clock(unsigned long long out[16], int reset)
{
    HIPCHK(hipDeviceSynchronize());
    static unsigned long long all[2048][16];
    HIPCHK(hipMemcpyFromSymbol(all, HIP_SYMBOL(g_phase_clock), sizeof all));
    for (int i = 0; i < 16; i++) { out[i] = 0; for (int b = 0; b < 2048; b++) out[i] += all[b][i]; }
    if (reset) { memset(all, 0, sizeof all); HIPCHK(hipMemcpyToSymbol(HIP_SYMBOL(g_phase_clock), all, sizeof all)); }
    return KAAMER_OK;
}
#endif

int kaamer_index_open_image(const kaamer_image *img, int device, kaamer_index **out)
{
    if (!img || !out) return kaamer_fail(KAAMER_E_ARG, "index_open_image: bad argument");
    *out = nullptr;
    HIPCHK(hipSetDevice(device));
    kaamer_index *ix = new (std::nothrow) kaamer_index();
    if (!ix) return kaamer_fail(KAAMER_E_NOMEM, "index alloc");
    ix->device = device;
    ix->n_top = 4;
    if (const char *e = getenv("KAAMER_HOST_SLOTS")) { const int v = atoi(e); if (v >= 1 && v <= KAAMER_MAX_HOST_SLOTS) ix->n_top = v; }
    ix->hdr = img->hdr;
    ix->d_buckets = nullptr;
    ix->d_arena = nullptr;
    int rc = dev_alloc(&ix->d_buckets, (size_t)img->hdr.n_buckets);
    if (!rc) rc = dev_alloc(&ix->d_arena, (size_t)(img->hdr.arena_words < 4 ? 4 : img->hdr.arena_words));
    if (rc) { kaamer_index_close(ix); return rc; }
    const kh_bucket *up_buckets = img->buckets;
    const uint32_t *up_arena = img->arena;
    std::vector<kh_bucket> ex_buckets;
    std::vector<uint32_t> ex_arena;
    if (const char *ev = getenv("KAAMER_EXP_ARENA_ORDER")) {
        struct Ref { uint32_t first_id, off; };
        std::vector<Ref> refs;
        const uint64_t nb = img->hdr.n_buckets;
        for (uint64_t b = 0; b < nb; b++)
            for (int t = 0; t < KH_SLOTS_PER_BUCKET; t++) {
                const kh_slot &sl = img->buckets[b].s[t];
                if (sl.key != KH_EMPTY_KEY && !(sl.val & KH_INLINE_BIT) && sl.val) refs.push_back(Ref{ img->arena[(uint64_t)sl.val * 4 + 1], sl.val });
            }
        std::sort(refs.begin(), refs.end(), [](const Ref &a, const Ref &b) { return a.off < b.off; });
        refs.erase(std::unique(refs.begin(), refs.end(), [](const Ref &a, const Ref &b) { return a.off == b.off; }), refs.end());
        if (atoi(ev) == 1) std::stable_sort(refs.begin(), refs.end(), [](const Ref &a, const Ref &b) { return a.first_id < b.first_id; });
        ex_arena.assign((size_t)img->hdr.arena_words, 0u);
        std::vector<uint32_t> new_off((size_t)(img->hdr.arena_words / 4 + 1), 0u);
        uint32_t cur = 1;
        for (const Ref &r : refs) {
            const uint32_t cnt = img->arena[(uint64_t)r.off * 4];
            const uint32_t units = (1u + cnt + 3u) / 4u;
            memcpy(&ex_arena[(size_t)cur * 4], &img->arena[(size_t)r.off * 4], (size_t)units * 16);
            new_off[r.off] = cur;
            cur += units;
        }
        ex_buckets.assign(img->buckets, img->buckets + nb);
        for (uint64_t b = 0; b < nb; b++)
            for (int t = 0; t < KH_SLOTS_PER_BUCKET; t++) {
                kh_slot &sl = ex_buckets[b].s[t];
                if (sl.key != KH_EMPTY_KEY && !(sl.val & KH_INLINE_BIT) && sl.val) sl.val = new_off[sl.val];
            }
        fprintf(stderr, "[kaamer experiment] arena re-ordered (%zu lists, %u units of %llu)\n", refs.size(), cur, (unsigned long long)(img->hdr.arena_words / 4));
        up_buckets = ex_buckets.data();
        up_arena = ex_arena.data();
    }
    hipError_t e = hipMemcpy(ix->d_buckets, up_buckets, (size_t)img->hdr.n_buckets * sizeof(kh_bucket), hipMemcpyHostToDevice);
    if (e == hipSuccess) e = hipMemcpy(ix->d_arena, up_arena, (size_t)img->hdr.arena_words * 4, hipMemcpyHostToDevice);
    if (e == hipSuccess) e = hipMemset(ix->d_arena, 0, 16);
    if (e != hipSuccess) { kaamer_index_close(ix); return kaamer_fail(KAAMER_E_HIP, "index upload: %s", hipGetErrorString(e)); }
    *out = ix;
    return KAAMER_OK;
}

int kaamer_index_build_proteins(const uint8_t *seqs, const uint64_t *offsets, const uint32_t *ids, uint32_t n_proteins,
                                uint32_t shard, uint32_t n_shards, double load_factor, int device, kaamer_index **out)
{
    if (!out || !offsets || (!seqs && n_proteins) || n_shards == 0 || shard >= n_shards)
        return kaamer_fail(KAAMER_E_ARG, "index_build_proteins: bad argument");
    *out = nullptr;
    kaamer_device_image di;
    const int rc = kaamer_build_on_device(seqs, offsets, ids, n_proteins, shard, n_shards, load_factor, device, &di);
    if (rc) return rc;
    kaamer_index *ix = new (std::nothrow) kaamer_index();
    if (!ix) { (void)hipFree(di.d_buckets); (void)hipFree(di.d_arena); return kaamer_fail(KAAMER_E_NOMEM, "index alloc"); }
    ix->device = device;
    ix->n_top = 4;
    if (const char *e = getenv("KAAMER_HOST_SLOTS")) { const int v = atoi(e); if (v >= 1 && v <= KAAMER_MAX_HOST_SLOTS) ix->n_top = v; }
    ix->hdr = di.hdr;
    ix->d_buckets = di.d_buckets;
    ix->d_arena = di.d_arena;
    *out = ix;
    return KAAMER_OK;
}

int kaamer_index_open(const char *path, int device, kaamer_index **out)
{
    kaamer_image *img = nullptr;
    int rc = kaamer_image_load(path, &img);
    if (rc) return rc;
    rc = kaamer_index_open_image(img, device, out);
    kaamer_image_free(img);
    return rc;
}

void kaamer_index_close(kaamer_index *ix)
{
    if (!ix) return;
    (void)hipSetDevice(ix->device);
    {
        std::unique_lock<std::mutex> lock(ix->pool_mu);
        for (;;) {
            bool busy = false;
            for (const HostSlot &h : ix->host) busy = busy || h.busy;
            for (int i = 0; i < ix->n_top; i++) busy = busy || ix->top[i].busy;
            if (!busy) break;
            ix->pool_cv.wait(lock);
        }
    }
    for (TopSlot &h : ix->top) if (h.stream) (void)hipStreamSynchronize(h.stream);
    for (HostSlot &h : ix->host) {
        if (h.stream) (void)hipStreamSynchronize(h.stream);
        if (h.stream) (void)hipStreamDestroy(h.stream);
        if (h.ws) kaamer_workspace_free(h.ws);
        if (h.d_seqs) (void)hipFree(h.d_seqs);
        if (h.d_off) (void)hipFree(h.d_off);
    }
    for (TopSlot &h : ix->top) top_slot_free(h);
    if (ix->d_buckets) (void)hipFree(ix->d_buckets);
    if (ix->d_arena) (void)hipFree(ix->d_arena);
    delete ix;
}

int kaamer_index_get_stats(const kaamer_index *ix, kaamer_image_stats *out)
{
    if (!ix || !out) return kaamer_fail(KAAMER_E_ARG, "index_get_stats: bad argument");
    kaamer_stats_from_header(&ix->hdr, out);
    return KAAMER_OK;
}

void kaamer_workspace_free(kaamer_workspace *ws)
{
    if (!ws) return;
    (void)hipSetDevice(ws->device);
    void *bufs[] = { ws->d_q, ws->d_nq, ws->d_n_pos, ws->d_valid, ws->d_vals, ws->d_cnt3, ws->d_off3, ws->d_n6, ws->d_long_seq, ws->d_long_np, ws->d_pcnt3, ws->d_n_piece_items, ws->d_piece_li, ws->d_piece_base, ws->d_poff3,
                     ws->d_tmp_meta, ws->d_orf_aa, ws->d_starts_alt, ws->d_q_cnt, ws->d_csr_off, ws->d_c_pid, ws->d_c_km, ws->d_c_fp,
                     ws->d_pool_cursor, ws->d_lists, ws->d_list_counts, ws->d_status_out, ws->d_qinfo, ws->d_slots,
                     ws->d_slot_off, ws->d_group_first, ws->d_n_groups, ws->d_pos_words, ws->d_pos_base, ws->d_pos_off, ws->d_pos_bits, ws->d_g_keys,
                     ws->d_counter_replicas, ws->d_counters, ws->d_bsum, ws->d_chain, ws->d_tr_chain, ws->d_sched, ws->d_n_sched, ws->d_group_start, ws->d_lay_total, ws->d_slot_scale, ws->d_top_cnt, ws->d_top_pid, ws->d_top_km, ws->d_top_fp, ws->d_top_trim, ws->d_top_start, ws->d_top_size, ws->d_rep_flag, ws->d_rep_aalen, ws->d_rep_query, ws->d_rep_pid, ws->d_rep_km, ws->d_rep_fp, ws->d_rep_trim, ws->d_rep_rank, ws->d_rep_eoff, ws->d_rep_aoff, ws->d_rep_off, ws->d_rep_q, ws->d_rep_aa, ws->d_hit_off,
                     ws->d_hit_pid, ws->d_hit_km, ws->d_hit_fp, ws->d_x_dst_off, ws->d_x_src_off, ws->d_x_nq_owned, ws->d_x_pid, ws->d_x_km, ws->d_x_fp, ws->d_x_ent_off, ws->d_x_tiles, ws->d_x_stats,
                     ws->d_x_dst_boff, ws->d_x_src_boff, ws->d_x_ent_boff, ws->d_x_mdst, ws->d_x_msize, ws->d_x_mbits, ws->d_x_gtab, ws->d_x_pstats };
    for (void *b : bufs) if (b) (void)hipFree(b);
    if (ws->h_x_stats) {
        (void)hipHostFree(ws->h_x_stats);
        for (hipEvent_t e : ws->ev_x_stats) if (e) (void)hipEventDestroy(e);
    }
    if (ws->ev) {
        for (hipEvent_t e : *ws->ev) (void)hipEventDestroy(e);
        delete ws->ev;
    }
    delete ws;
}

int kaamer_workspace_create(kaamer_index *ix, const kaamer_workspace_opts *opts, kaamer_workspace **out)
{
    if (!ix || !opts || !out) return kaamer_fail(KAAMER_E_ARG, "workspace_create: bad argument");
    *out = nullptr;
    HIPCHK(hipSetDevice(ix->device));
    kaamer_workspace *ws = new (std::nothrow) kaamer_workspace();
    if (!ws) return kaamer_fail(KAAMER_E_NOMEM, "workspace alloc");
    memset(ws, 0, sizeof *ws);
    ws->device = ix->device;
    ws->opts = *opts;
    ws->nucleotide = opts->seq_type == KAAMER_NUCLEOTIDE || opts->seq_type == KAAMER_READS;
    ws->max_seqs = opts->max_seqs ? opts->max_seqs : 1;
    if (ws->nucleotide) {
        ws->aa_cap = 2 * opts->max_seq_bytes + 64;
        ws->sa_cap = ws->aa_cap;
        uint64_t qc = opts->max_queries ? opts->max_queries : (uint64_t)ws->max_seqs * 4 + opts->max_seq_bytes / 32 + 64;
        if (qc > 0xFFFFFFF0ull) qc = 0xFFFFFFF0ull;
        ws->q_cap = (uint32_t)qc;
        ws->pos_cap = ws->aa_cap + 64;
    } else {
        ws->q_cap = opts->max_queries > ws->max_seqs ? opts->max_queries : ws->max_seqs;
        ws->pos_cap = opts->max_seq_bytes + 64;
    }
    if (ws->q_cap < 1) ws->q_cap = 1;
    ws->hit_cap = opts->max_hits ? opts->max_hits : std::min<uint64_t>((uint64_t)ws->q_cap * 256, ws->pos_cap) + (1u << 20);
    ws->g_slots = opts->g_tier_slots ? opts->g_tier_slots : (32ull << 20);
    {
        const uint64_t items = ws->pos_cap > ws->hit_cap ? ws->pos_cap : ws->hit_cap;
        ws->sparse_cap = items + items / 2 + 64ull * ws->q_cap + GRP_MAX_TABLE + ws->hit_cap / 2 + (1u << 20);
    }
    ws->firstpos = opts->first_pos == 1 || (opts->first_pos == 0 && (opts->seq_type == KAAMER_NUCLEOTIDE || opts->seq_type == KAAMER_READS));
    int grp_per_cu = 0, p_per_cu = 0;
    ws->count_async = false;
    if (const char *e = getenv("KAAMER_COUNT_ASYNC")) ws->count_async = atoi(e) != 0;
    hipError_t oe = ws->count_async
        ? (ws->firstpos ? hipOccupancyMaxActiveBlocksPerMultiprocessor(&grp_per_cu, count_async_kernel<true>, 64 * GRP_WAVES, 0)
                        : hipOccupancyMaxActiveBlocksPerMultiprocessor(&grp_per_cu, count_async_kernel<false>, 64 * GRP_WAVES, 0))
        : (ws->firstpos ? hipOccupancyMaxActiveBlocksPerMultiprocessor(&grp_per_cu, count_group_kernel<true, 0>, 64 * GRP_WAVES, 0)
                        : hipOccupancyMaxActiveBlocksPerMultiprocessor(&grp_per_cu, count_group_kernel<false, 0>, 64 * GRP_WAVES, 0));
    if (oe == hipSuccess)
        oe = ws->nucleotide ? hipOccupancyMaxActiveBlocksPerMultiprocessor(&p_per_cu, probe_kernel<true>, 64 * P_WAVES, 0)
                  : hipOccupancyMaxActiveBlocksPerMultiprocessor(&p_per_cu, probe_kernel<false>, 64 * P_WAVES, 0);
    if (oe != hipSuccess) { delete ws; return kaamer_fail(KAAMER_E_HIP, "occupancy query: %s", hipGetErrorString(oe)); }
    hipDeviceProp_t prop;
    hipError_t pe = hipGetDeviceProperties(&prop, ix->device);
    if (pe != hipSuccess) { delete ws; return kaamer_fail(KAAMER_E_HIP, "hipGetDeviceProperties: %s", hipGetErrorString(pe)); }
    if (grp_per_cu < 1) grp_per_cu = 1;
    if (p_per_cu < 1) p_per_cu = 1;
    if (opts->concurrent_batches > 1 && !ws->nucleotide) grp_per_cu = 1;
    ws->sched_identity = false;
    if (const char *e = getenv("KAAMER_SCHED_IDENTITY")) ws->sched_identity = atoi(e) != 0;
    if (const char *e = getenv("KAAMER_GRP_PER_CU")) { const int v = atoi(e); if (v >= 1 && v <= 3) grp_per_cu = v < grp_per_cu || opts->concurrent_batches > 1 ? v : grp_per_cu; }
    if (const char *e = getenv("KAAMER_P_PER_CU")) { const int v = atoi(e); if (v >= 1 && v < p_per_cu) p_per_cu = v; }
    ws->n_cu = prop.multiProcessorCount;
    ws->grp_grid = ws->n_cu * grp_per_cu;
    {
        int g_per_cu = 0;
        if (hipOccupancyMaxActiveBlocksPerMultiprocessor(&g_per_cu, count_global_kernel, 64 * G_WAVES, 0) != hipSuccess || g_per_cu < 1) g_per_cu = 1;
        ws->g_grid = ws->n_cu * (g_per_cu > 2 ? 2 : g_per_cu);
    }
    ws->p_grid = ws->n_cu * p_per_cu;
    {
        int pk_per_cu = 0;
        hipError_t ke = ws->nucleotide ? hipOccupancyMaxActiveBlocksPerMultiprocessor(&pk_per_cu, count_pack_kernel<true, PK_ARENA_ORF>, 64, 0)
                        : ws->firstpos ? hipOccupancyMaxActiveBlocksPerMultiprocessor(&pk_per_cu, count_pack_kernel<true, PK_ARENA_PROT>, 64, 0)
                                       : hipOccupancyMaxActiveBlocksPerMultiprocessor(&pk_per_cu, count_pack_kernel<false, PK_ARENA_PROT>, 64, 0);
        if (ke != hipSuccess || pk_per_cu < 1) pk_per_cu = 1;
        if (const char *e = getenv("KAAMER_PACK_PER_CU")) { const int v = atoi(e); if (v >= 1 && v < pk_per_cu) pk_per_cu = v; }
        ws->pack_grid = ws->n_cu * pk_per_cu;
        int pl = 0;
        if (hipOccupancyMaxActiveBlocksPerMultiprocessor(&pl, count_pack_kernel<true, PK_ARENA_ORF_LONG>, 64, 0) != hipSuccess || pl < 1) pl = 1;
        ws->pack_grid_long = ws->n_cu * pl;
    }
    ws->pack_shift = 9u;
    if (const char *e = getenv("KAAMER_PACK_SHIFT")) { const int v = atoi(e); if (v >= 8 && v <= 10) ws->pack_shift = (uint32_t)v; }
    ws->use_group = !ws->nucleotide;
    if (getenv("KAAMER_COUNT_GROUP")) ws->use_group = true;
    if (getenv("KAAMER_COUNT_PACK")) ws->use_group = false;
    ws->unit_windows = 2;
    if (const char *e = getenv("KAAMER_UNIT_WINDOWS")) { const int v = atoi(e); if (v == 2 || (v == 4 && grp_per_cu == 1)) ws->unit_windows = v; }
    if (ws->use_group) ws->pack_shift = ws->count_async ? GRP_SHIFT : ws->unit_windows == 4 ? GRP_SHIFT + 2u : GRP_SHIFT + 1u;
    if (const char *e = getenv("KAAMER_GROUP_SHIFT")) { const int v = atoi(e); if (ws->use_group && !ws->count_async && ws->unit_windows == 2 && (v == (int)GRP_SHIFT || v == (int)GRP_SHIFT + 1)) ws->pack_shift = (uint32_t)v; }
    {
        const uint64_t items = ws->pos_cap > ws->hit_cap ? ws->pos_cap : ws->hit_cap;
        const uint64_t gc = (((uint64_t)GRP_MIN_TABLE * ws->q_cap + 3 * items) >> 8) + 4;
        ws->groups_cap = (uint32_t)(gc > 0x7FFFFFFFull ? 0x7FFFFFFFull : gc);
    }
    int rc = KAAMER_OK;
    {
        uint64_t n = ws->q_cap;
        if (ws->nucleotide && (uint64_t)ws->max_seqs * 6 > n) n = (uint64_t)ws->max_seqs * 6;
        if (ws->nucleotide) {
            const uint64_t ml = opts->max_seq_bytes / (TS_MAX + 1) + 1;
            ws->max_long = (uint32_t)(ml < ws->max_seqs ? ml : ws->max_seqs);
            ws->max_piece_items = 6ull * (opts->max_seq_bytes / 3 / TP_PIECE + ws->max_long + 1);
            if (ws->max_piece_items > n) n = ws->max_piece_items;
        }
        ws->n_scan_blocks = (uint32_t)((n + 1 + SCAN_TILE - 1) / SCAN_TILE);
    }
    rc = dev_alloc(&ws->d_q, ws->q_cap);
    if (!rc) rc = dev_alloc(&ws->d_nq, 1);
    if (!rc) rc = dev_alloc(&ws->d_n_pos, 1);
    if (!rc) rc = dev_alloc(&ws->d_valid, (size_t)(ws->pos_cap / 64 + 2));
    if (!rc) rc = dev_alloc(&ws->d_vals, (size_t)ws->pos_cap);
    if (!rc && ws->nucleotide) {
        const size_t n6 = (size_t)ws->max_seqs * 6;
        rc = dev_alloc(&ws->d_cnt3, 3 * n6);
        if (!rc) rc = dev_alloc(&ws->d_off3, 3 * (n6 + 1));
        if (!rc) rc = dev_alloc(&ws->d_n6, 1);
        if (!rc) rc = dev_alloc(&ws->d_long_seq, (size_t)ws->max_long + 1);
        if (!rc) rc = dev_alloc(&ws->d_piece_li, (size_t)ws->max_piece_items / 6 + 2);
        if (!rc) rc = dev_alloc(&ws->d_long_np, (size_t)ws->max_long + 1);
        if (!rc) rc = dev_alloc(&ws->d_piece_base, (size_t)ws->max_long + 2);
        if (!rc) rc = dev_alloc(&ws->d_pcnt3, 3 * (size_t)ws->max_piece_items);
        if (!rc) rc = dev_alloc(&ws->d_poff3, 3 * ((size_t)ws->max_piece_items + 1));
        if (!rc) rc = dev_alloc(&ws->d_n_piece_items, 1);
        if (!rc) rc = dev_alloc(&ws->d_tmp_meta, ws->q_cap);
        const size_t tcw = 3 * ((size_t)ws->max_seqs / 64 + 2);
        if (!rc) rc = dev_alloc(&ws->d_tr_chain, tcw);
        if (!rc && hipMemset(ws->d_tr_chain, 0, tcw * sizeof(unsigned long long)) != hipSuccess) rc = kaamer_fail(KAAMER_E_HIP, "memset");
        if (!rc) rc = dev_alloc(&ws->d_orf_aa, (size_t)ws->aa_cap + 64);
        if (!rc) rc = dev_alloc(&ws->d_starts_alt, (size_t)ws->sa_cap + 64);
    }
    if (!rc) rc = dev_alloc(&ws->d_q_cnt, ws->q_cap);
    if (!rc) rc = dev_alloc(&ws->d_pool_cursor, (size_t)3 * CURSOR_STRIDE);
    if (!rc) rc = dev_alloc(&ws->d_lists, (size_t)N_LISTS * ws->q_cap);
    if (!rc) rc = dev_alloc(&ws->d_list_counts, N_SMALL_SLOTS);
    if (!rc) rc = dev_alloc(&ws->d_status_out, 1);
    if (!rc) rc = dev_alloc(&ws->d_qinfo, ws->q_cap);
    if (!rc) rc = dev_alloc(&ws->d_slots, ws->q_cap);
    if (!rc) rc = dev_alloc(&ws->d_slot_off, (size_t)ws->q_cap + 1);
    if (!rc) rc = dev_alloc(&ws->d_group_first, ws->groups_cap);
    if (!rc) rc = dev_alloc(&ws->d_sched, ws->groups_cap);
    if (!rc) rc = dev_alloc(&ws->d_group_start, ws->groups_cap);
    if (!rc) rc = dev_alloc(&ws->d_lay_total, 1);
    if (!rc) rc = dev_alloc(&ws->d_slot_scale, 4);
    if (!rc) {
        const uint32_t one = SLOT_SCALE_ONE;
        if (hipMemcpy(ws->d_slot_scale, &one, 4, hipMemcpyHostToDevice) != hipSuccess) rc = kaamer_fail(KAAMER_E_HIP, "workspace init");
        ws->table_room = (unsigned long long)(0.7 * (double)ws->sparse_cap);
        double cap = 128.0;
        if (getenv("KAAMER_SLOT_SCALE_MAX")) cap = atof(getenv("KAAMER_SLOT_SCALE_MAX")) * 16.0;
        ws->slot_scale_cap = cap < 16.0 ? 16u : cap > 128.0 ? 128u : (uint32_t)cap;
        ws->slot_scale_margin = 30u;
        ws->dense_tables = getenv("KAAMER_PACK_LONG") != nullptr;
        if (getenv("KAAMER_SLOT_MARGIN")) ws->slot_scale_margin = (uint32_t)(atof(getenv("KAAMER_SLOT_MARGIN")) * 16.0);
        if (getenv("KAAMER_WS_TRACE"))
            fprintf(stderr, "[kaamer workspace] pos_cap %llu q_cap %u hit_cap %llu sparse_cap %llu table_room %llu slot_scale_cap %u/16\n", (unsigned long long)ws->pos_cap,
                    ws->q_cap, (unsigned long long)ws->hit_cap, (unsigned long long)ws->sparse_cap, ws->table_room, ws->slot_scale_cap);
    }
    if (!rc) rc = dev_alloc(&ws->d_n_sched, 1);
    if (!rc) rc = dev_alloc(&ws->d_n_groups, 1);

    ws->want_positions = opts->want_positions != 0;
    if (!rc && ws->want_positions) {
        ws->bits_cap = opts->max_pos_words ? opts->max_pos_words : ws->hit_cap * 8;
        rc = dev_alloc(&ws->d_pos_words, ws->q_cap);
        if (!rc) rc = dev_alloc(&ws->d_pos_base, (size_t)ws->q_cap + 1);
        if (!rc) rc = dev_alloc(&ws->d_pos_off, ws->sparse_cap);
        if (!rc) rc = dev_alloc(&ws->d_pos_bits, ws->bits_cap);
    }
    if (!rc) rc = dev_alloc(&ws->d_g_keys, 4 * ws->g_slots);
    if (!rc) rc = dev_alloc(&ws->d_counter_replicas, (size_t)CTR_REPLICAS * CTR_N);
    if (!rc) rc = dev_alloc(&ws->d_counters, 1);
    if (!rc) rc = dev_alloc(&ws->d_bsum, ws->n_scan_blocks);
    if (!rc) rc = dev_alloc(&ws->d_chain, (size_t)ws->q_cap / PL_TILE + 2);
    if (!rc && hipMemset(ws->d_chain, 0, ((size_t)ws->q_cap / PL_TILE + 2) * sizeof(unsigned long long)) != hipSuccess) rc = kaamer_fail(KAAMER_E_HIP, "memset");
    if (!rc) rc = dev_alloc(&ws->d_hit_off, (size_t)ws->q_cap + 1);
    ws->compact = opts->compact != 0;
    if (!rc) rc = dev_alloc(&ws->d_hit_pid, ws->sparse_cap);
    if (!rc) rc = dev_alloc(&ws->d_hit_km, ws->sparse_cap);
    if (!rc) rc = dev_alloc(&ws->d_hit_fp, ws->sparse_cap);
    if (!rc && !ws->firstpos && hipMemset(ws->d_hit_fp, 0, ws->sparse_cap * sizeof(uint32_t)) != hipSuccess) rc = kaamer_fail(KAAMER_E_HIP, "memset");
    if (!rc && ws->compact) {
        rc = dev_alloc(&ws->d_csr_off, (size_t)ws->q_cap + 1);
        if (!rc) rc = dev_alloc(&ws->d_c_pid, ws->hit_cap);
        if (!rc) rc = dev_alloc(&ws->d_c_km, ws->hit_cap);
        if (!rc) rc = dev_alloc(&ws->d_c_fp, ws->hit_cap);
        if (!rc && !ws->firstpos && hipMemset(ws->d_c_fp, 0, ws->hit_cap * sizeof(uint32_t)) != hipSuccess) rc = kaamer_fail(KAAMER_E_HIP, "memset");
    }
    if (rc) { kaamer_workspace_free(ws); return rc; }
    ws->ev = new (std::nothrow) std::vector<hipEvent_t>();
    if (!ws->ev) { kaamer_workspace_free(ws); return kaamer_fail(KAAMER_E_NOMEM, "event ring"); }
    *out = ws;
    return KAAMER_OK;
}

static void launch_layout(kaamer_workspace *ws, uint32_t nq_bound, uint32_t *status, hipStream_t s, uint32_t bshift, bool schedule = true)
{
    const uint32_t cshift = bshift > GRP_SHIFT ? 10u : bshift >= GRP_SHIFT ? 9u : 7u;
    ws->lay_epoch = (ws->lay_epoch + 1u) & 0xFFFFFFu;
    if (ws->lay_epoch == 0) ws->lay_epoch = 1;
    const uint32_t tiles = (uint32_t)(((uint64_t)nq_bound + 1 + LAY_TILE - 1) / LAY_TILE);
    hipLaunchKernelGGL(layout_kernel, dim3(tiles), dim3(LAY_THREADS), 0, s, ws->d_slots, ws->d_nq, ws->d_slot_off, ws->d_group_first,
                       ws->d_group_start, ws->d_n_groups, ws->groups_cap, ws->d_chain, ws->lay_epoch, status, bshift);
    if (schedule)
        hipLaunchKernelGGL(schedule_kernel, dim3(1), dim3(1024), 0, s, ws->d_group_first, ws->d_group_start, ws->d_slot_off, ws->d_n_groups,
                           ws->d_nq, ws->d_sched, ws->d_n_sched, cshift);
}

static void launch_pos_layout(kaamer_workspace *ws, uint32_t nq_bound, const int32_t *sizes, uint32_t *status, hipStream_t s)
{
    uint32_t gb = (nq_bound + 255) / 256;
    if (gb < 1) gb = 1;
    if (gb > (uint32_t)ws->n_cu * 8) gb = (uint32_t)ws->n_cu * 8;
    hipLaunchKernelGGL(pos_words_kernel, dim3(gb), dim3(256), 0, s, ws->d_qinfo, sizes, ws->d_q_cnt, ws->d_nq, ws->d_pos_words);
    if (nq_bound <= 8 * SCAN_TILE) {
        hipLaunchKernelGGL(scan_single_kernel, dim3(1), dim3(SCAN_BLOCK), 0, s, ws->d_pos_words, ws->d_nq, ws->d_pos_base);
    } else {
        const uint32_t nsb = (uint32_t)(((uint64_t)nq_bound + 1 + SCAN_TILE - 1) / SCAN_TILE);
        hipLaunchKernelGGL(scan_block_sums_kernel, dim3(nsb), dim3(SCAN_BLOCK), 0, s, ws->d_pos_words, ws->d_nq, ws->d_bsum);
        hipLaunchKernelGGL(scan_top_kernel, dim3(1), dim3(SCAN_BLOCK), 0, s, ws->d_bsum, nsb);
        hipLaunchKernelGGL(scan_apply_kernel, dim3(nsb), dim3(SCAN_BLOCK), 0, s, ws->d_pos_words, ws->d_nq, ws->d_bsum, ws->d_pos_base);
    }
    hipLaunchKernelGGL(pos_layout_kernel, dim3(ws->n_cu * 8), dim3(256), 0, s, ws->d_qinfo, sizes, ws->d_q_cnt,
                       ws->compact ? ws->d_csr_off : ws->d_hit_off,
                       ws->d_pos_base, ws->d_nq, ws->d_pos_off, ws->d_pos_bits, ws->bits_cap, status);
}

static void launch_compaction(kaamer_workspace *ws, uint32_t nq_bound, uint32_t *status, hipStream_t s)
{
    if (nq_bound <= 8 * SCAN_TILE) {
        hipLaunchKernelGGL(scan_single_kernel, dim3(1), dim3(SCAN_BLOCK), 0, s, ws->d_q_cnt, ws->d_nq, ws->d_csr_off);
    } else {
        const uint32_t nsb = (uint32_t)(((uint64_t)nq_bound + 1 + SCAN_TILE - 1) / SCAN_TILE);
        hipLaunchKernelGGL(scan_block_sums_kernel, dim3(nsb), dim3(SCAN_BLOCK), 0, s, ws->d_q_cnt, ws->d_nq, ws->d_bsum);
        hipLaunchKernelGGL(scan_top_kernel, dim3(1), dim3(SCAN_BLOCK), 0, s, ws->d_bsum, nsb);
        hipLaunchKernelGGL(scan_apply_kernel, dim3(nsb), dim3(SCAN_BLOCK), 0, s, ws->d_q_cnt, ws->d_nq, ws->d_bsum, ws->d_csr_off);
    }
    uint32_t gb = (nq_bound + 3) / 4;
    if (gb < 1) gb = 1;
    if (gb > (uint32_t)ws->n_cu * 8) gb = (uint32_t)ws->n_cu * 8;
    hipLaunchKernelGGL(gather_hits_kernel, dim3(gb), dim3(256), 0, s, ws->d_nq, ws->d_csr_off, ws->d_hit_off, ws->d_q_cnt, ws->d_hit_pid,
                       ws->d_hit_km, ws->d_hit_fp, ws->d_c_pid, ws->d_c_km, ws->d_c_fp, ws->hit_cap, status, 1);
}

static void fill_result_hits(const kaamer_workspace *ws, kaamer_device_result *out)
{
    out->d_hit_cnt = ws->d_q_cnt;
    out->hit_capacity = ws->compact ? ws->hit_cap : ws->sparse_cap;
    out->d_hit_off = ws->compact ? ws->d_csr_off : ws->d_hit_off;
    out->d_hit_pid = ws->compact ? ws->d_c_pid : ws->d_hit_pid;
    out->d_hit_kmatch = ws->compact ? ws->d_c_km : ws->d_hit_km;
    out->d_hit_first_pos = ws->compact ? ws->d_c_fp : ws->d_hit_fp;
}

static int ws_join(kaamer_workspace *ws, hipStream_t stream)
{
    if (ws->split_pending && ws->count_stream && ws->count_stream != stream) HIPCHK(hipStreamWaitEvent(stream, ws->ev_count, 0));
    return KAAMER_OK;
}

int kaamer_workspace_set_count_stream(kaamer_workspace *ws, void *stream)
{
    if (!ws) return kaamer_fail(KAAMER_E_ARG, "workspace_set_count_stream: bad argument");
    HIPCHK(hipSetDevice(ws->device));
    if (ws->split_pending) HIPCHK(hipEventSynchronize(ws->ev_count));
    ws->split_pending = false;
    ws->count_stream = (hipStream_t)stream;
    if (stream && !ws->ev_probe) {
        HIPCHK(hipEventCreateWithFlags(&ws->ev_probe, hipEventDisableTiming));
        HIPCHK(hipEventCreateWithFlags(&ws->ev_count, hipEventDisableTiming));
    }
    return KAAMER_OK;
}

int kaamer_search_device(kaamer_index *ix, kaamer_workspace *ws, const uint8_t *d_seqs, const uint64_t *d_offsets,
                         uint32_t n_seqs, uint64_t seq_bytes, int32_t seq_type, void *stream,
                         kaamer_device_result *out)
{
    if (!ix || !ws || !out || (n_seqs && (!d_seqs || !d_offsets))) return kaamer_fail(KAAMER_E_ARG, "search_device: bad argument");
    if (ix->device != ws->device) return kaamer_fail(KAAMER_E_ARG, "workspace belongs to another device");
    const bool nucl = seq_type == KAAMER_NUCLEOTIDE || seq_type == KAAMER_READS;
    if (!nucl && seq_type != KAAMER_PROTEIN) return kaamer_fail(KAAMER_E_ARG, "search_device: unknown sequence type %d", seq_type);
    if (nucl != ws->nucleotide) return kaamer_fail(KAAMER_E_ARG, "workspace was created for %s input", ws->nucleotide ? "nucleotide" : "protein");
    if (n_seqs > ws->max_seqs) return kaamer_fail(KAAMER_E_CAPACITY, "batch of %u sequences exceeds workspace max_seqs %u", n_seqs, ws->max_seqs);
    if (ws->pos_cap > 0xFFFFFFF0ull) return kaamer_fail(KAAMER_E_CAPACITY, "a batch holds at most 2^32 residue positions");
    if (seq_bytes > ws->opts.max_seq_bytes) return kaamer_fail(KAAMER_E_CAPACITY, "batch of %llu bytes exceeds workspace max_seq_bytes", (unsigned long long)seq_bytes);
    hipStream_t s = (hipStream_t)stream;
    HIPCHK(hipSetDevice(ix->device));
    {
        const int jrc = ws_join(ws, s);
        if (jrc) return jrc;
        ws->split_pending = false;
    }
    const bool timed = ws->time_every && (ws->call_no++ % ws->time_every) == 0;
    hipEvent_t *ev = nullptr;
    if (timed) {
        if (ws->n_timed >= MAX_TIMED_CALLS) ws->n_timed = 0;
        while (ws->ev->size() < (size_t)(ws->n_timed + 1) * EV_PER_CALL) {
            hipEvent_t e;
            HIPCHK(hipEventCreate(&e));
            ws->ev->push_back(e);
        }
        ev = ws->ev->data() + (size_t)ws->n_timed * EV_PER_CALL;
        HIPCHK(hipEventRecord(ev[0], s));
    }
    if (!ws->clean) {
        HIPCHK(hipMemsetAsync(ws->d_pool_cursor, 0, (size_t)3 * CURSOR_STRIDE * sizeof(unsigned long long), s));
        HIPCHK(hipMemsetAsync(ws->d_list_counts, 0, N_SMALL_SLOTS * sizeof(uint32_t), s));
        HIPCHK(hipMemsetAsync(ws->d_counter_replicas, 0, sizeof(unsigned long long) * CTR_REPLICAS * CTR_N, s));
        HIPCHK(hipMemsetAsync(ws->d_valid, 0, (size_t)(ws->pos_cap / 64 + 2) * sizeof(unsigned long long), s));
    }
    ws->clean = false;

    uint32_t *status = ws->d_list_counts + SLOT_STATUS;
    uint32_t *queue_head = ws->d_list_counts + SLOT_QUEUE_HEAD;
    const int pb = 256;
    const uint8_t *residues = d_seqs;
    uint64_t pos_bound = seq_bytes;
    uint32_t nq_bound = n_seqs;
    if (!nucl) {
        PrepLayoutParams pl;
        memset(&pl, 0, sizeof pl);
        pl.seqs = d_seqs; pl.pos_bound = seq_bytes; pl.offsets = d_offsets; pl.n_seqs = n_seqs;
        pl.q = ws->d_q; pl.d_nq = ws->d_nq; pl.d_n_pos = ws->d_n_pos; pl.invalid = ws->d_valid; pl.qinfo = ws->d_qinfo;
        pl.hit_off = ws->d_hit_off; pl.q_cnt = ws->d_q_cnt;
        pl.E = ws->d_slot_off; pl.group_first = ws->d_group_first; pl.group_start = ws->d_group_start;
        pl.d_n_groups = ws->d_n_groups; pl.groups_cap = ws->groups_cap; pl.chain = ws->d_chain;
        ws->lay_epoch = (ws->lay_epoch + 1u) & 0xFFFFFFu;
        if (ws->lay_epoch == 0) ws->lay_epoch = 1;
        pl.epoch = ws->lay_epoch;
        pl.status = status; pl.sched = ws->d_sched; pl.d_n_sched = ws->d_n_sched;
        pl.tiles_done = ws->d_list_counts + SLOT_TILES_DONE;
        pl.slots = ws->d_slots; pl.bshift = ws->pack_shift; pl.cshift = ws->pack_shift > GRP_SHIFT ? 10u : ws->pack_shift >= GRP_SHIFT ? 9u : 7u;
        pl.no_sched = (ws->use_group && !ws->sched_identity) ? 0u : 1u;
        pl.d_total = ws->d_lay_total;
        pl.slot_scale = ws->d_slot_scale;
        pl.room_slots = ws->table_room;
        const uint32_t tiles = (uint32_t)(((uint64_t)n_seqs + 1 + PL_TILE - 1) / PL_TILE);
        hipLaunchKernelGGL(prep_layout_schedule_kernel, dim3(tiles), dim3(LAY_THREADS), 0, s, pl);
    } else {
        const size_t cap6 = (size_t)ws->max_seqs * 6;
        TranslateParams tp;
        memset(&tp, 0, sizeof tp);
        tp.seqs = d_seqs; tp.offsets = d_offsets; tp.n_seqs = n_seqs; tp.seq_bound = seq_bytes; tp.max_long = ws->max_long; tp.max_piece_items = ws->max_piece_items;
        tp.cnt_orf = ws->d_cnt3; tp.cnt_aa = ws->d_cnt3 + cap6; tp.cnt_sa = ws->d_cnt3 + 2 * cap6;
        tp.off_orf = ws->d_off3; tp.off_aa = ws->d_off3 + (cap6 + 1); tp.off_sa = ws->d_off3 + 2 * (cap6 + 1);
        tp.tmp_meta = ws->d_tmp_meta; tp.orf_aa = ws->d_orf_aa; tp.starts_alt = ws->d_starts_alt;
        tp.q_cap = ws->q_cap; tp.aa_cap = ws->aa_cap; tp.sa_cap = ws->sa_cap; tp.status = status;
        bool wide_reads = seq_bytes > 160ull * (n_seqs ? n_seqs : 1u);
        if (const char *e = getenv("KAAMER_WIDE_READS")) wide_reads = atoi(e) != 0;
        tp.ts_max = wide_reads ? TS_MAX_WIDE : TS_MAX;
        int tgrid = ws->n_cu * 8;
        tp.d_n6 = ws->d_n6;
        int sgrid = ws->n_cu * 8;
        if ((uint64_t)sgrid * TS_WAVES * 64 > (uint64_t)n_seqs) sgrid = n_seqs > 0 ? (int)(((uint64_t)n_seqs + TS_WAVES * 64 - 1) / (TS_WAVES * 64)) : 1;
        tp.n_long = ws->d_list_counts + SLOT_N_LONG;
        const size_t mpi = (size_t)ws->max_piece_items;
        tp.long_seq = ws->d_long_seq; tp.long_np = ws->d_long_np; tp.piece_base = ws->d_piece_base; tp.piece_li = ws->d_piece_li;
        tp.pcnt_orf = ws->d_pcnt3; tp.pcnt_aa = ws->d_pcnt3 + mpi; tp.pcnt_sa = ws->d_pcnt3 + 2 * mpi;
        tp.poff_orf = ws->d_poff3; tp.poff_aa = ws->d_poff3 + (mpi + 1); tp.poff_sa = ws->d_poff3 + 2 * (mpi + 1);
        tp.d_n_piece_items = ws->d_n_piece_items;
        auto scan_u32 = [&](const uint32_t *cnt, const uint32_t *d_count, uint64_t bound, uint64_t *off) {
            if (bound <= 8 * (uint64_t)SCAN_TILE) {
                hipLaunchKernelGGL(scan_single_kernel, dim3(1), dim3(SCAN_BLOCK), 0, s, cnt, d_count, off);
            } else {
                const uint32_t nsb = (uint32_t)((bound + 1 + SCAN_TILE - 1) / SCAN_TILE);
                hipLaunchKernelGGL(scan_block_sums_kernel, dim3(nsb), dim3(SCAN_BLOCK), 0, s, cnt, d_count, ws->d_bsum);
                hipLaunchKernelGGL(scan_top_kernel, dim3(1), dim3(SCAN_BLOCK), 0, s, ws->d_bsum, nsb);
                hipLaunchKernelGGL(scan_apply_kernel, dim3(nsb), dim3(SCAN_BLOCK), 0, s, cnt, d_count, ws->d_bsum, off);
            }
        };
        const uint64_t long_bound = (uint64_t)ws->max_long < n_seqs ? ws->max_long : n_seqs;
        const uint64_t seq_long_max = seq_bytes / (TS_MAX + 1) + 1;
        const uint64_t n_long_bound = long_bound < seq_long_max ? long_bound : seq_long_max;
        const uint64_t piece_bound = 6ull * (seq_bytes / 3 / TP_PIECE + n_long_bound + 1);
        if ((uint64_t)tgrid * 4 > piece_bound) tgrid = (int)((piece_bound + 3) / 4);
        if (tgrid < 1) tgrid = 1;
        tp.ticket = ws->d_list_counts + SLOT_TR_TICKET;
        tp.chain = ws->d_tr_chain;
        ws->tr_epoch = (ws->tr_epoch + 1u) & 0xFFFFFFu;
        if (ws->tr_epoch == 0) ws->tr_epoch = 1;
        tp.epoch = ws->tr_epoch;
        tp.out_meta = ws->d_q; tp.d_nq = ws->d_nq; tp.d_n_pos = ws->d_n_pos;
        tp.w_off_orf = ws->d_off3; tp.w_off_aa = ws->d_off3 + (cap6 + 1); tp.w_off_sa = ws->d_off3 + 2 * (cap6 + 1);
        hipLaunchKernelGGL(list_long_kernel, dim3((unsigned)(((uint64_t)n_seqs + LL_BLOCK - 1) / LL_BLOCK + (n_seqs ? 0 : 1))), dim3(LL_BLOCK), 0, s, tp);
        scan_u32(ws->d_long_np, tp.n_long, n_long_bound, ws->d_piece_base);
        hipLaunchKernelGGL(piece_li_kernel, dim3((unsigned)((n_long_bound + 255) / 256)), dim3(256), 0, s, tp);
        hipLaunchKernelGGL(translate_kernel<false>, dim3(tgrid), dim3(256), 0, s, tp);
        for (int a = 0; a < 3; a++) scan_u32(ws->d_pcnt3 + a * mpi, ws->d_n_piece_items, piece_bound, ws->d_poff3 + a * (mpi + 1));
        hipLaunchKernelGGL(long_totals_kernel, dim3((unsigned)((n_long_bound * 6 + 255) / 256)), dim3(256), 0, s, tp);
        if (wide_reads) hipLaunchKernelGGL(translate_reads_kernel<TS_MAX_WIDE>, dim3(sgrid), dim3(64 * TS_WAVES), 0, s, tp);
        else hipLaunchKernelGGL(translate_reads_kernel<TS_MAX>, dim3(sgrid), dim3(64 * TS_WAVES), 0, s, tp);
        hipLaunchKernelGGL(translate_kernel<true>, dim3(tgrid), dim3(256), 0, s, tp);
        hipLaunchKernelGGL(orf_order_long_kernel, dim3((unsigned)(n_long_bound < (uint64_t)ws->n_cu * 32 ? (n_long_bound + 3) / 4 + 1 : (uint64_t)ws->n_cu * 8)), dim3(256), 0, s,
                           ws->d_tmp_meta, tp.off_orf, ws->d_long_seq, tp.n_long, ws->d_q, ws->d_nq);
        hipLaunchKernelGGL(prep_orf_kernel, dim3(ws->n_cu * 4), dim3(pb), 0, s, ws->d_q, ws->d_nq, ws->d_valid, ws->d_n_pos,
                           ws->d_qinfo, ws->d_slots, ws->d_hit_off, ws->d_q_cnt, ws->d_slot_scale, ws->table_room);
        residues = ws->d_orf_aa;
        pos_bound = ws->aa_cap;
        nq_bound = ws->q_cap;
    }

    if (nucl) launch_layout(ws, nq_bound, status, s, ws->pack_shift, ws->use_group);

    ProbeParams pp;
    pp.table = reinterpret_cast<const uint4 *>(ix->d_buckets);
    pp.n_buckets = ix->hdr.n_buckets;
    pp.n_shards = ix->hdr.n_shards;
    pp.shard = ix->hdr.shard;
    pp.residues = residues;
    pp.invalid = ws->d_valid;
    pp.d_n_pos = ws->d_n_pos;
    pp.vals = ws->d_vals;
    pp.counters = ws->d_counter_replicas;
    pp.nontemporal = pos_bound < ix->hdr.n_buckets ? 1u : 0u;
    uint64_t p_blocks = (pos_bound / 64 + 1 + P_WAVES - 1) / P_WAVES;
    if (p_blocks > (uint64_t)ws->p_grid) p_blocks = ws->p_grid;
    if (p_blocks < 1) p_blocks = 1;
    if (timed) HIPCHK(hipEventRecord(ev[1], s));
    if (ws->nucleotide) hipLaunchKernelGGL(probe_kernel<true>, dim3((unsigned)p_blocks), dim3(64 * P_WAVES), 0, s, pp);
    else hipLaunchKernelGGL(probe_kernel<false>, dim3((unsigned)p_blocks), dim3(64 * P_WAVES), 0, s, pp);
    if (timed) HIPCHK(hipEventRecord(ev[2], s));
    const bool split = ws->count_stream && ws->count_stream != s && !timed;
    if (split) {
        HIPCHK(hipEventRecord(ws->ev_probe, s));
        HIPCHK(hipStreamWaitEvent(ws->count_stream, ws->ev_probe, 0));
        s = ws->count_stream;
    }
    CountParams p;
    memset(&p, 0, sizeof p);
    p.arena = ix->d_arena;
    p.vals = ws->d_vals;
    p.qinfo = ws->d_qinfo;
    p.slot_off = ws->d_slot_off;
    p.group_first = ws->d_group_first;
    p.sched = ws->d_sched;
    p.d_n_sched = ws->d_n_sched;
    p.d_n_groups = ws->d_n_groups;
    p.d_nq = ws->d_nq;
    p.list_cap = ws->q_cap;
    p.queue_head = queue_head;
    p.group_queue = ws->d_list_counts + SLOT_GROUP_QUEUE;
    p.hit_off = ws->d_hit_off;
    p.q_cnt = ws->d_q_cnt;
    p.hit_pid = ws->d_hit_pid;
    p.hit_km = ws->d_hit_km;
    p.hit_fp = ws->d_hit_fp;
    p.hit_cap = ws->sparse_cap;
    p.tail_cursor = ws->d_pool_cursor;
    p.g_keys = ws->d_g_keys;
    p.g_slots = ws->g_slots;
    p.g_cursor = ws->d_pool_cursor + CURSOR_STRIDE;
    p.n_proteins = ix->hdr.max_protein_id + 1u ? ix->hdr.max_protein_id + 1u : 0xFFFFFFFFu;
    p.counters = ws->d_counter_replicas;
    p.status = status;
    auto list_ptr = [&](int which) { return ws->d_lists + (size_t)which * ws->q_cap; };

    CountParams pc = p;
    pc.ovf_list = list_ptr(LIST_G); pc.ovf_count = ws->d_list_counts + LIST_G;
    pc.last_group_pass = ws->want_positions ? 0u : 1u;
    pc.pack_shift = ws->pack_shift;
    pc.pack_tickets = ws->d_list_counts + SLOT_PACK_TICKETS;
    {
        uint64_t gb = (((uint64_t)GRP_MIN_TABLE * nq_bound + 3 * pos_bound) >> ws->pack_shift) + 1;
        if (gb > (uint64_t)ws->pack_grid) gb = ws->pack_grid;
        if (ws->use_group) {
            uint64_t gg = ((uint64_t)GRP_MIN_TABLE * nq_bound + 3 * pos_bound) / GRP_BUDGET + 1;
            if (gg > (uint64_t)ws->grp_grid) gg = ws->grp_grid;
            launch_group(pc, (int)gg, ws->firstpos, s, ws->count_async, ws->unit_windows);
        } else if (ws->nucleotide) {
            const bool long_orfs = seq_bytes > 200ull * (n_seqs ? n_seqs : 1u) || ws->dense_tables;
            uint64_t g2 = gb;
            if (long_orfs) {
                if (g2 > (uint64_t)ws->pack_grid_long) g2 = ws->pack_grid_long;
                hipLaunchKernelGGL((count_pack_kernel<true, PK_ARENA_ORF_LONG>), dim3((unsigned)g2), dim3(64), 0, s, pc);
            } else {
                hipLaunchKernelGGL((count_pack_kernel<true, PK_ARENA_ORF>), dim3((unsigned)g2), dim3(64), 0, s, pc);
            }
        }
        else if (ws->firstpos) hipLaunchKernelGGL((count_pack_kernel<true, PK_ARENA_PROT>), dim3((unsigned)gb), dim3(64), 0, s, pc);
        else hipLaunchKernelGGL((count_pack_kernel<false, PK_ARENA_PROT>), dim3((unsigned)gb), dim3(64), 0, s, pc);
    }
    CountParams pg = p;
    pg.list = list_ptr(LIST_G); pg.list_count = ws->d_list_counts + LIST_G;
    int g_grid = ws->g_grid;
    if ((uint32_t)g_grid > nq_bound) g_grid = nq_bound > 0 ? (int)nq_bound : 1;
    const bool fused_finalize = !ws->compact && !ws->want_positions;
    if (fused_finalize) {
        pg.fin_out = ws->d_counters; pg.fin_small = ws->d_list_counts; pg.fin_status_out = ws->d_status_out;
        pg.fin_cursors = ws->d_pool_cursor;
        pg.fin_slot_scale = ws->d_slot_scale; pg.fin_scale_cap = ws->slot_scale_cap; pg.fin_scale_margin = ws->slot_scale_margin;
    }
    hipLaunchKernelGGL(count_global_kernel, dim3(g_grid), dim3(64 * G_WAVES), 0, s, pg);
    if (ws->compact) launch_compaction(ws, nq_bound, status, s);
    if (timed) HIPCHK(hipEventRecord(ev[3], s));

    if (ws->want_positions) {
        launch_pos_layout(ws, nq_bound, nullptr, status, s);
        launch_layout(ws, nq_bound, status, s, GRP_SHIFT);
        uint64_t grp_blocks = ((uint64_t)GRP_MIN_TABLE * nq_bound + 3 * pos_bound) / GRP_BUDGET + 1;
        if (grp_blocks > (uint64_t)ws->grp_grid) grp_blocks = ws->grp_grid;
        CountParams pp2 = p;
        pp2.pack_shift = GRP_SHIFT;
        pp2.last_group_pass = 1u;
        pp2.pos_base = ws->d_pos_base;
        pp2.pos_bits = ws->d_pos_bits;
        pp2.group_queue = ws->d_list_counts + SLOT_GROUP_QUEUE_POS;
        pp2.ovf_list = list_ptr(LIST_SO); pp2.ovf_count = ws->d_list_counts + LIST_SO;
        launch_group_positions(pp2, (int)grp_blocks, s);
        CountParams pg2 = pg;
        pg2.fin_out = nullptr;
        pg2.pos_base = ws->d_pos_base;
        pg2.pos_bits = ws->d_pos_bits;
        pg2.g_cursor = ws->d_pool_cursor + 2 * CURSOR_STRIDE;
        hipLaunchKernelGGL(positions_global_kernel, dim3(g_grid), dim3(64 * G_WAVES), 0, s, pg2);
    }
    if (!fused_finalize)
        hipLaunchKernelGGL(finalize_kernel, dim3(1), dim3(256), 0, s, ws->d_counter_replicas, ws->d_counters, ws->d_list_counts,
                           ws->d_status_out, ws->d_pool_cursor, ws->d_slot_scale, ws->slot_scale_cap, ws->slot_scale_margin);
    if (timed) HIPCHK(hipEventRecord(ev[4], s));
    HIPCHK(hipGetLastError());
    if (split) {
        HIPCHK(hipEventRecord(ws->ev_count, s));
        ws->split_pending = true;
    }
    ws->clean = true;
    ws->last_was_merge = false;
    if (timed) ws->n_timed++;

    out->n_queries_cap = ws->q_cap;
    out->d_n_queries = ws->d_nq;
    out->d_q = ws->d_q;
    fill_result_hits(ws, out);
    out->d_orf_aa = nucl ? ws->d_orf_aa : nullptr;
    out->d_starts_alt = nucl ? ws->d_starts_alt : nullptr;
    out->d_counters = ws->d_counters;
    out->d_pos_off = ws->want_positions ? ws->d_pos_off : nullptr;
    out->d_pos_bits = ws->want_positions ? (const uint64_t *)ws->d_pos_bits : nullptr;
    out->d_pos_base = ws->want_positions ? ws->d_pos_base : nullptr;
    return KAAMER_OK;
}

static int merge_device_impl(kaamer_workspace *ws, const uint64_t *d_ent_off, const uint32_t *d_pid, const uint32_t *d_km,
                             const uint32_t *d_fp, uint32_t n_queries, const uint32_t *d_n_queries, uint64_t n_entries, void *stream,
                             kaamer_device_result *out, XParams *xpos = nullptr)
{
    if (!ws || !out || (n_queries && !d_ent_off) || (n_entries && (!d_pid || !d_km || !d_fp)))
        return kaamer_fail(KAAMER_E_ARG, "merge_device: bad argument");
    if (n_queries > ws->q_cap) return kaamer_fail(KAAMER_E_CAPACITY, "merge of %u queries exceeds the workspace (%u)", n_queries, ws->q_cap);
    if (n_entries > ws->hit_cap) return kaamer_fail(KAAMER_E_CAPACITY, "merge of %llu entries exceeds workspace max_hits", (unsigned long long)n_entries);
    hipStream_t s = (hipStream_t)stream;
    HIPCHK(hipSetDevice(ws->device));
    if (!ws->clean) {
        HIPCHK(hipMemsetAsync(ws->d_pool_cursor, 0, (size_t)3 * CURSOR_STRIDE * sizeof(unsigned long long), s));
        HIPCHK(hipMemsetAsync(ws->d_list_counts, 0, N_SMALL_SLOTS * sizeof(uint32_t), s));
        HIPCHK(hipMemsetAsync(ws->d_counter_replicas, 0, sizeof(unsigned long long) * CTR_REPLICAS * CTR_N, s));
        HIPCHK(hipMemsetAsync(ws->d_valid, 0, (size_t)(ws->pos_cap / 64 + 2) * sizeof(unsigned long long), s));
    }
    ws->clean = false;
    uint32_t *status = ws->d_list_counts + SLOT_STATUS;
    const uint32_t nq_bound = n_queries;
    const int pb = 256;
    hipLaunchKernelGGL(prep_merge_kernel, dim3((n_queries + pb - 1) / pb > 0 ? (n_queries + pb - 1) / pb : 1), dim3(pb), 0, s, d_ent_off,
                       n_queries, d_n_queries, ws->d_qinfo, ws->d_slots, ws->d_nq, ws->d_hit_off, ws->d_q_cnt);
    launch_layout(ws, nq_bound, status, s, GRP_SHIFT + 1u);
    CountParams p;
    memset(&p, 0, sizeof p);
    p.qinfo = ws->d_qinfo;
    p.slot_off = ws->d_slot_off;
    p.group_first = ws->d_group_first;
    p.sched = ws->d_sched;
    p.d_n_sched = ws->d_n_sched;
    p.d_n_groups = ws->d_n_groups;
    p.d_nq = ws->d_nq;
    p.last_group_pass = 1u;
    p.pack_shift = GRP_SHIFT + 1u;
    p.group_queue = ws->d_list_counts + SLOT_GROUP_QUEUE;
    p.m_pid = d_pid; p.m_km = d_km; p.m_fp = d_fp; p.merge_fp = ws->firstpos ? 1u : 0u;
    p.list_cap = ws->q_cap;
    p.hit_off = ws->d_hit_off;
    p.q_cnt = ws->d_q_cnt;
    p.hit_pid = ws->d_hit_pid; p.hit_km = ws->d_hit_km; p.hit_fp = ws->d_hit_fp;
    p.hit_cap = ws->sparse_cap;
    p.tail_cursor = ws->d_pool_cursor;
    p.g_keys = ws->d_g_keys;
    p.g_slots = ws->g_slots;
    p.g_cursor = ws->d_pool_cursor + CURSOR_STRIDE;
    p.counters = ws->d_counter_replicas;
    p.status = status;
    auto list_ptr = [&](int which) { return ws->d_lists + (size_t)which * ws->q_cap; };
    p.ovf_list = list_ptr(LIST_G); p.ovf_count = ws->d_list_counts + LIST_G;
    {
        uint64_t gb = ((uint64_t)GRP_MIN_TABLE * nq_bound + 3 * n_entries) / GRP_BUDGET + 1;
        if (gb > (uint64_t)ws->grp_grid) gb = ws->grp_grid;
        launch_group_merge(p, (int)gb, ws->firstpos, s);
    }
    CountParams pg = p;
    pg.list = list_ptr(LIST_G); pg.list_count = ws->d_list_counts + LIST_G;
    int g_grid = ws->g_grid;
    if ((uint32_t)g_grid > nq_bound) g_grid = nq_bound > 0 ? (int)nq_bound : 1;
    hipLaunchKernelGGL(merge_global_kernel, dim3(g_grid), dim3(256), 0, s, pg);
    if (ws->compact) launch_compaction(ws, nq_bound, status, s);
    if (xpos) {
        launch_pos_layout(ws, nq_bound, xpos->m_size, status, s);
        xpos->r_nq = ws->d_nq;
        xpos->r_cnt = ws->d_q_cnt;
        xpos->r_off = ws->compact ? ws->d_csr_off : ws->d_hit_off;
        xpos->r_pid = ws->compact ? ws->d_c_pid : ws->d_hit_pid;
        xpos->r_pos_off = ws->d_pos_off;
        xpos->r_pos_base = ws->d_pos_base;
        xpos->r_pos_bits = ws->d_pos_bits;
        xpos->r_bits_cap = ws->bits_cap;
        uint32_t gb = nq_bound < (uint32_t)ws->n_cu * 16 ? nq_bound : (uint32_t)ws->n_cu * 16;
        hipLaunchKernelGGL(x_or_bits_kernel, dim3(gb ? gb : 1), dim3(64), 0, s, *xpos);
    }
    hipLaunchKernelGGL(finalize_kernel, dim3(1), dim3(256), 0, s, ws->d_counter_replicas, ws->d_counters, ws->d_list_counts,
                       ws->d_status_out, ws->d_pool_cursor, (uint32_t *)nullptr, 16u, 16u);
    HIPCHK(hipGetLastError());
    ws->clean = true;
    ws->last_was_merge = true;
    memset(out, 0, sizeof *out);
    out->n_queries_cap = ws->q_cap;
    out->d_n_queries = ws->d_nq;
    fill_result_hits(ws, out);
    out->d_counters = ws->d_counters;
    if (xpos) {
        out->d_pos_off = ws->d_pos_off;
        out->d_pos_bits = (const uint64_t *)ws->d_pos_bits;
        out->d_pos_base = ws->d_pos_base;
    }
    return KAAMER_OK;
}

int kaamer_merge_device(kaamer_workspace *ws, const uint64_t *d_ent_off, const uint32_t *d_pid, const uint32_t *d_km,
                        const uint32_t *d_fp, uint32_t n_queries, uint64_t n_entries, void *stream, kaamer_device_result *out)
{
    return merge_device_impl(ws, d_ent_off, d_pid, d_km, d_fp, n_queries, nullptr, n_entries, stream, out);
// ... 835 lines not shown
```

Measured before the change: 25.87 billion.

## Fuse k-mer hash probing into async count kernel and skip separate probe pass

For protein, single-shard, no-position runs, the standalone probe kernel is dropped. The count_async kernel now builds k-mer keys from residues through an LDS lookup table and probes the hash table inside its software pipeline, using an extra pipeline stage to hide probe latency. Overflow queries handled by the global kernel probe inline and write vals. The invalid bitmap marking is skipped. This removes the round trip that writes the vals array and reads it back, and one kernel launch. In exchange the fused kernel holds more live state and is capped at lower occupancy (4 blocks) through launch bounds.

New measurement: 25.74 billion, median of 2. Within noise of the previous version (-0.5%).

```diff
diff --git a/kaamer_amd/csrc/count_async.hip.inc b/kaamer_amd/csrc/count_async.hip.inc
--- a/kaamer_amd/csrc/count_async.hip.inc
+++ b/kaamer_amd/csrc/count_async.hip.inc
@@ -3,9 +3,12 @@
 #define CA_ARENA (GRP_BUDGET - 64u + GRP_MAX_TABLE)
 #define CA_NONE 0xFFFFFFFFu
 #define GRP_WQ 64u
-
-template <bool FIRSTPOS>
-__global__ __launch_bounds__(64 * GRP_WAVES, FIRSTPOS ? 5 : 6) void count_async_kernel(CountParams p)
+#ifndef CA_FUSED_WAVES
+#define CA_FUSED_WAVES 4
+#endif
+
+template <bool FIRSTPOS, bool FUSED>
+__global__ __launch_bounds__(64 * GRP_WAVES, FUSED ? CA_FUSED_WAVES : FIRSTPOS ? 5 : 6) void count_async_kernel(CountParams p)
 {
     constexpr int WAVES = GRP_WAVES;
     constexpr int XIT = 2;
@@ -33,8 +36,9 @@
     __shared__ uint32_t s_hint;
     __shared__ uint32_t s_pref[WAVES][64];
     __shared__ uint8_t s_own[WAVES][XIT * 64];
-    __shared__ unsigned long long s_tot[8];
-    enum { T_IN = 0, T_Q, T_POST, T_HITS, T_OVF, T_LISTS, T_LIDS };
+    __shared__ unsigned long long s_tot[10];
+    __shared__ uint8_t s_lut[FUSED ? 256 : 1];
+    enum { T_IN = 0, T_Q, T_POST, T_HITS, T_OVF, T_LISTS, T_LIDS, T_LOOKUP, T_PROBE, T_FOUND };
 
     const uint32_t tid = threadIdx.x, lane = tid & 63u, wv = tid >> 6;
 #ifdef KAAMER_PHASE_CLOCK
@@ -63,7 +67,9 @@
         return make_uint2(uni(e.x), uni(e.y));
     };
 
-    if (tid < 8) s_tot[tid] = 0;
+    if (tid < 10) s_tot[tid] = 0;
+    if (FUSED)
+        for (uint32_t i = tid; i < 256; i += 64 * WAVES) s_lut[i] = (uint8_t)kh_residue_code((uint8_t)i);
     for (uint32_t i = tid; i < WAVES * XIT * 64; i += 64 * WAVES) (&s_own[0][0])[i] = 0;
     for (uint32_t i = tid; i < CA_ARENA; i += 64 * WAVES) {
         a_keys[i] = KH_EMPTY_PID;
@@ -312,7 +318,7 @@
             my_k++;
         }
     };
-    struct RawA { uint32_t vraw, j, ps; };
+    struct RawA { uint32_t vraw, j, ps; KmerWords kw; };
     auto issue_a = [&](const Job &jb) {
         RawA r;
         const uint32_t c = jb.c, w = jb.w;
@@ -332,13 +338,20 @@
         }
         r.j = j;
         r.ps = valid ? i - c_pref[c][j] : 0u;
-        r.vraw = p.vals[valid ? c_aa[c][j] + r.ps : 0ull];
+        if (FUSED) {
+            r.vraw = 0u;
+            r.kw = kmer_words(p.residues, valid ? c_aa[c][j] + r.ps : 0ull);
+        } else {
+            r.vraw = p.vals[valid ? c_aa[c][j] + r.ps : 0ull];
+            r.kw.w0 = r.kw.w1 = r.kw.w2 = r.kw.sh = 0u;
+        }
         return r;
     };
     auto lane_valid = [&](const Job &jb) { return jb.valid != 0u && ((jb.w << 6) + lane) < jb.npos; };
     auto issue_b = [&](uint32_t v) { return reinterpret_cast<const uint4 *>(p.arena)[(v & KH_INLINE_BIT) ? 0u : v]; };
 
     uint32_t c_post = 0, c_lists = 0, c_lids = 0;
+    uint32_t c_lookup = 0, c_probe = 0, c_found = 0;
     uint32_t *const pref = s_pref[wv];
     uint8_t *const own = s_own[wv];
     auto add_n = [&](uint32_t c, uint32_t j, uint32_t pid, uint32_t pos, uint32_t n) {
@@ -456,11 +469,18 @@
         if (uni(got)) build(1u);
     }
 
-    Job j0, j1;
+    Job j0, j1, jb;
     j0.valid = j1.valid = 0u; j0.w = j1.w = 0u; j0.c = j1.c = 0u; j0.npos = j1.npos = 0u; j0.nq = j1.nq = 0u; j0.need = j1.need = CA_NONE;
-    RawA a0, a1;
+    jb = j0;
+    RawA a0, a1, ab;
     a0.vraw = a0.j = a0.ps = 0u;
+    a0.kw.w0 = a0.kw.w1 = a0.kw.w2 = a0.kw.sh = 0u;
     a1 = a0;
+    ab = a0;
+    BucketLoads bl1;
+    uint32_t key1 = KH_NO_KEY;
+#pragma unroll
+    for (int u = 0; u < 4; u++) { bl1.ld[u] = make_uint4(0, 0, 0, 0); bl1.rk[u] = KH_NO_KEY; }
     uint32_t v0 = 0;
     uint4 hv0 = make_uint4(0, 0, 0, 0);
     uint32_t tp = 0;
@@ -476,14 +496,25 @@
                 have_tp = true;
             }
             if (try_resolve(tp, j2)) have_tp = false;
-            else if (!j0.valid && !j1.valid) {
+            else if (!j0.valid && !j1.valid && !(FUSED && jb.valid)) {
                 if (!help()) { CA_CLK(ca_idle, __builtin_amdgcn_s_sleep(2)); if (++spins > (1u << 24)) { if (lane == 0) atomicOr(p.status, (uint32_t)ST_CHAIN_TIMEOUT); break; } }
                 continue;
             }
         }
-        if (at_end && !j0.valid && !j1.valid && !j2.valid) break;
+        if (at_end && !j0.valid && !j1.valid && !j2.valid && !(FUSED && jb.valid)) break;
         const RawA a2 = issue_a(j2);
-        const uint32_t v1 = lane_valid(j1) ? a1.vraw : 0u;
+        uint32_t v1;
+        BucketLoads blb;
+        uint32_t keyb = KH_NO_KEY;
+        if (FUSED) {
+            keyb = lane_valid(jb) ? kmer_key(ab.kw, s_lut) : KH_NO_KEY;
+            c_lookup += keyb != KH_NO_KEY ? 1u : 0u;
+            probe_issue<false>(p.table, 1u, p.n_buckets, p.nontemporal != 0u, keyb, 0u, blb);
+            v1 = probe_finish(p.table, 1u, p.n_buckets, p.nontemporal != 0u, bl1, key1, c_probe);
+            c_found += v1 != 0u ? 1u : 0u;
+        } else {
+            v1 = lane_valid(j1) ? a1.vraw : 0u;
+        }
         const uint4 hv1 = issue_b(v1);
         if (j0.valid) {
             const uint32_t c = j0.c;
@@ -501,8 +532,15 @@
             __builtin_amdgcn_fence(__ATOMIC_RELEASE, "workgroup", "local");
             if (lane == 0 && atomicAdd(&c_wdone[c], 1u) + 1u == (j0.npos + 63u) >> 6) atomicAdd(&s_hint, 1u);
         }
-        a0 = a1; v0 = v1; hv0 = hv1; a1 = a2;
-        j0 = j1; j1 = j2;
+        if (FUSED) {
+            c_probe += keyb != KH_NO_KEY ? 1u : 0u;
+            a0 = a1; v0 = v1; hv0 = hv1; a1 = ab; ab = a2;
+            bl1 = blb; key1 = keyb;
+            j0 = j1; j1 = jb; jb = j2;
+        } else {
+            a0 = a1; v0 = v1; hv0 = hv1; a1 = a2;
+            j0 = j1; j1 = j2;
+        }
         {
             const uint32_t h = uni(ld(&s_hint));
             if (h != seen_hint) { seen_hint = h; help(); }
@@ -517,6 +555,14 @@
             atomicAdd(&s_tot[T_POST], (unsigned long long)a);
             atomicAdd(&s_tot[T_LISTS], (unsigned long long)b);
             atomicAdd(&s_tot[T_LIDS], (unsigned long long)c);
+        }
+        if (FUSED) {
+            const uint32_t l = wave_total(c_lookup), pr = wave_total(c_probe), fo = wave_total(c_found);
+            if (lane == 0) {
+                atomicAdd(&s_tot[T_LOOKUP], (unsigned long long)l);
+                atomicAdd(&s_tot[T_PROBE], (unsigned long long)pr);
+                atomicAdd(&s_tot[T_FOUND], (unsigned long long)fo);
+            }
         }
     }
 #ifdef KAAMER_PHASE_CLOCK
@@ -536,6 +582,11 @@
         add_counter(p.counters, rep, CTR_OVERFLOW, s_tot[T_OVF]);
         add_counter(p.counters, rep, CTR_LISTS, s_tot[T_LISTS]);
         add_counter(p.counters, rep, CTR_LIST_IDS, s_tot[T_LIDS]);
+        if (FUSED) {
+            add_counter(p.counters, rep, CTR_LOOKUP, s_tot[T_LOOKUP]);
+            add_counter(p.counters, rep, CTR_PROBE, s_tot[T_PROBE]);
+            add_counter(p.counters, rep, CTR_FOUND, s_tot[T_FOUND]);
+        }
     }
 }
 #undef CA_CLK
diff --git a/kaamer_amd/csrc/count_group.hip.inc b/kaamer_amd/csrc/count_group.hip.inc
--- a/kaamer_amd/csrc/count_group.hip.inc
+++ b/kaamer_amd/csrc/count_group.hip.inc
@@ -222,6 +222,7 @@
     unsigned long long *d_total;
     const uint32_t *slot_scale;
     unsigned long long room_slots;
+    uint32_t no_bitmap;
 };
 
 #define PL_ITEMS 1
@@ -242,7 +243,7 @@
         if (batch_bad) atomicOr(p.status, (uint32_t)ST_AA_CAP);
         *p.d_nq = nq;
         *p.d_n_pos = n_pos;
-        mark_invalid_range(p.invalid, n_pos, (n_pos + 63) & ~63ull);
+        if (!p.no_bitmap) mark_invalid_range(p.invalid, n_pos, (n_pos + 63) & ~63ull);
     }
 #pragma unroll
     for (int r = 0; r < PL_ITEMS; r++) {
@@ -275,10 +276,10 @@
             qi.aa_off = b;
             if (size >= 7) {
                 qi.slots = table_slots_for(size, slot_scale);
-                mark_invalid_range(p.invalid, b + (uint64_t)size, e);
+                if (!p.no_bitmap) mark_invalid_range(p.invalid, b + (uint64_t)size, e);
             } else {
                 qi.slots = 0;
-                mark_invalid_range(p.invalid, b, e);
+                if (!p.no_bitmap) mark_invalid_range(p.invalid, b, e);
             }
             p.qinfo[i] = qi;
             p.slots[i] = qi.slots;
diff --git a/kaamer_amd/csrc/search.hip b/kaamer_amd/csrc/search.hip
--- a/kaamer_amd/csrc/search.hip
+++ b/kaamer_amd/csrc/search.hip
@@ -142,6 +142,101 @@
 #define P_WAVES 4
 #define P_RING 128u
 #define KH_NO_KEY 0xFFFFFFFDu
+
+struct BucketLoads {
+    uint4 ld[4];
+    uint32_t rk[4];
+};
+template <bool SKIP_IDLE>
+__device__ __forceinline__ void probe_issue(const uint4 *table, uint32_t n_shards, uint64_t n_buckets, bool nontemporal, uint32_t key,
+                                            uint32_t step, BucketLoads &b)
+{
+    const uint32_t lane = threadIdx.x & 63u;
+    const uint32_t nb = (uint32_t)n_buckets;
+    uint32_t my_bucket = 0u;
+    if (key != KH_NO_KEY) {
+        my_bucket = (uint32_t)kh_home_bucket(key, n_shards, n_buckets) + step;
+        my_bucket = my_bucket >= nb ? my_bucket - nb : my_bucket;
+    }
+#pragma unroll
+    for (int j = 0; j < 4; j++) {
+        const int src = 16 * j + (int)(lane >> 2);
+        b.rk[j] = __shfl(key, src, 64);
+        const uint32_t bucket = __shfl(my_bucket, src, 64);
+        typedef uint32_t v4u __attribute__((ext_vector_type(4)));
+        const v4u *srcp = reinterpret_cast<const v4u *>(table) + (uint64_t)bucket * 4 + (lane & 3u);
+        if (SKIP_IDLE) {
+            b.ld[j] = make_uint4(KH_EMPTY_KEY, 0u, KH_EMPTY_KEY, 0u);
+            if (b.rk[j] != KH_NO_KEY) {
+                const v4u t = *srcp;
+                b.ld[j] = make_uint4(t.x, t.y, t.z, t.w);
+            }
+        } else {
+            const v4u t = nontemporal ? __builtin_nontemporal_load(srcp) : *srcp;
+            b.ld[j] = make_uint4(t.x, t.y, t.z, t.w);
+        }
+    }
+}
+__device__ __forceinline__ void probe_consume(const BucketLoads &b, uint32_t &okey, uint32_t &oval, uint32_t &oempty)
+{
+    const uint32_t lane = threadIdx.x & 63u;
+    okey = KH_NO_KEY; oval = 0; oempty = 1u;
+#pragma unroll
+    for (int j = 0; j < 4; j++) {
+        const uint32_t kk = b.rk[j];
+        const uint4 &l = b.ld[j];
+        uint32_t r = (l.x == kk) ? l.y : ((l.z == kk) ? l.w : 0u);
+        uint32_t e = (l.x == KH_EMPTY_KEY || l.z == KH_EMPTY_KEY) ? 1u : 0u;
+        r |= (uint32_t)__builtin_amdgcn_update_dpp(0, (int)r, 0xB1, 0xf, 0xf, false);
+        e |= (uint32_t)__builtin_amdgcn_update_dpp(0, (int)e, 0xB1, 0xf, 0xf, false);
+        r |= (uint32_t)__builtin_amdgcn_update_dpp(0, (int)r, 0x4E, 0xf, 0xf, false);
+        e |= (uint32_t)__builtin_amdgcn_update_dpp(0, (int)e, 0x4E, 0xf, 0xf, false);
+        const bool take = (lane & 3u) == (uint32_t)j;
+        okey = take ? kk : okey; oval = take ? r : oval; oempty = take ? e : oempty;
+    }
+}
+__device__ __forceinline__ uint32_t probe_finish(const uint4 *table, uint32_t n_shards, uint64_t n_buckets, bool nontemporal,
+                                                 const BucketLoads &b, uint32_t key, uint32_t &extra)
+{
+    const uint32_t lane = threadIdx.x & 63u;
+    const int owner = (int)(4u * (lane & 15u) + (lane >> 4));
+    uint32_t okey, oval, oempty;
+    probe_consume(b, okey, oval, oempty);
+    uint32_t v = __shfl(oval, owner, 64), e = __shfl(oempty, owner, 64);
+    uint32_t step = 0;
+    bool more = key != KH_NO_KEY && v == 0u && e == 0u && 1u < n_buckets;
+    while (__ballot(more)) {
+        step++;
+        extra += more ? 1u : 0u;
+        BucketLoads d;
+        probe_issue<true>(table, n_shards, n_buckets, nontemporal, more ? key : KH_NO_KEY, step, d);
+        probe_consume(d, okey, oval, oempty);
+        const uint32_t v2 = __shfl(oval, owner, 64), e2 = __shfl(oempty, owner, 64);
+        v = more ? v2 : v;
+        more = more && v2 == 0u && e2 == 0u && step + 1u < n_buckets;
+    }
+    return v;
+}
+struct KmerWords {
+    uint32_t w0, w1, w2, sh;
+};
+__device__ __forceinline__ KmerWords kmer_words(const uint8_t *residues, uint64_t at)
+{
+    const uintptr_t a = (uintptr_t)(residues + at);
+    const uint32_t *w = reinterpret_cast<const uint32_t *>(a & ~(uintptr_t)3);
+    KmerWords k;
+    k.sh = (uint32_t)(a & 3u);
+    k.w0 = w[0];
+    k.w1 = w[1];
+    k.w2 = w[k.sh >= 2u ? 2 : 1];
+    return k;
+}
+__device__ __forceinline__ uint32_t kmer_key(const KmerWords &k, const uint8_t *lut)
+{
+    const uint32_t lo = __builtin_amdgcn_alignbyte(k.w1, k.w0, k.sh), hi = __builtin_amdgcn_alignbyte(k.w2, k.w1, k.sh);
+    return kh_key_from_codes(lut[lo & 0xFFu], lut[(lo >> 8) & 0xFFu], lut[(lo >> 16) & 0xFFu], lut[lo >> 24], lut[hi & 0xFFu],
+                             lut[(hi >> 8) & 0xFFu], lut[(hi >> 16) & 0xFFu]);
+}
 
 template <bool SKIP_IDLE> __global__ __launch_bounds__(64 * P_WAVES) void probe_kernel(ProbeParams p)
 {
@@ -206,44 +301,10 @@
         if (!ring) w += stride;
         fetch(w, mask, ra, rb);
 
-        uint32_t my_bucket = 0u;
-        if (key != KH_NO_KEY) {
-            my_bucket = (uint32_t)kh_home_bucket(key, p.n_shards, p.n_buckets) + step;
-            my_bucket = my_bucket >= n_buckets ? my_bucket - n_buckets : my_bucket;
-        }
-        uint4 ld[4];
-        uint32_t rk[4];
-#pragma unroll
-        for (int j = 0; j < 4; j++) {
-            const int src = 16 * j + (int)(lane >> 2);
-            rk[j] = __shfl(key, src, 64);
-            const uint32_t bucket = __shfl(my_bucket, src, 64);
-            typedef uint32_t v4u __attribute__((ext_vector_type(4)));
-            const v4u *srcp = reinterpret_cast<const v4u *>(p.table) + (uint64_t)bucket * 4 + (lane & 3u);
-            if (SKIP_IDLE) {
-                ld[j] = make_uint4(KH_EMPTY_KEY, 0u, KH_EMPTY_KEY, 0u);
-                if (rk[j] != KH_NO_KEY) {
-                    const v4u t = *srcp;
-                    ld[j] = make_uint4(t.x, t.y, t.z, t.w);
-                }
-            } else {
-                const v4u t = p.nontemporal ? __builtin_nontemporal_load(srcp) : *srcp;
-                ld[j] = make_uint4(t.x, t.y, t.z, t.w);
-            }
-        }
-        uint32_t okey = KH_NO_KEY, oval = 0, oempty = 1u;
-#pragma unroll
-        for (int j = 0; j < 4; j++) {
-            const uint32_t kk = rk[j];
-            uint32_t r = (ld[j].x == kk) ? ld[j].y : ((ld[j].z == kk) ? ld[j].w : 0u);
-            uint32_t e = (ld[j].x == KH_EMPTY_KEY || ld[j].z == KH_EMPTY_KEY) ? 1u : 0u;
-            r |= (uint32_t)__builtin_amdgcn_update_dpp(0, (int)r, 0xB1, 0xf, 0xf, false);
-            e |= (uint32_t)__builtin_amdgcn_update_dpp(0, (int)e, 0xB1, 0xf, 0xf, false);
-            r |= (uint32_t)__builtin_amdgcn_update_dpp(0, (int)r, 0x4E, 0xf, 0xf, false);
-            e |= (uint32_t)__builtin_amdgcn_update_dpp(0, (int)e, 0x4E, 0xf, 0xf, false);
-            const bool take = (lane & 3u) == (uint32_t)j;
-            okey = take ? kk : okey; oval = take ? r : oval; oempty = take ? e : oempty;
-        }
+        BucketLoads bl;
+        probe_issue<SKIP_IDLE>(p.table, p.n_shards, p.n_buckets, p.nontemporal != 0u, key, step, bl);
+        uint32_t okey, oval, oempty;
+        probe_consume(bl, okey, oval, oempty);
         const uint32_t ooff = __shfl(off, (int)mine, 64);
         const bool valid = okey != KH_NO_KEY;
         c_found += (valid && oval != 0u) ? 1u : 0u;
@@ -278,6 +339,11 @@
 struct CountParams {
     const uint32_t *arena;
     const uint32_t *vals;
+    const uint4 *table;
+    uint64_t n_buckets;
+    const uint8_t *residues;
+    uint32_t *vals_out;
+    uint32_t nontemporal;
     const struct QInfo *qinfo;
     const uint64_t *slot_off;
     uint32_t *group_first;
@@ -669,12 +735,15 @@
     __shared__ uint32_t s_roff[G_MAX_RANGES], s_rcur[G_MAX_RANGES], s_rtotal;
     __shared__ LongSink s_long;
     __shared__ uint32_t b_keys[BigLdsTable::CAP], b_val[BigLdsTable::CAP];
+    __shared__ uint8_t s_lut[256];
 
     const uint32_t tid = threadIdx.x, lane = tid & 63u, wv = tid >> 6;
     const uint32_t n_items = *p.list_count < p.list_cap ? *p.list_count : p.list_cap;
     const uint32_t n_part = n_items < gridDim.x ? (n_items ? n_items : 1u) : gridDim.x;
     if (blockIdx.x >= n_part) return;
     unsigned long long tot_hits = 0, f_post = 0, f_lists = 0, f_lids = 0, mon_hits = 0;
+    if (p.vals_out)
+        for (uint32_t i = tid; i < 256; i += 64 * WAVES) s_lut[i] = (uint8_t)kh_residue_code((uint8_t)i);
     uint32_t mon_q = 0;
 #ifdef KAAMER_PHASE_CLOCK
     unsigned long long gq_acc[10] = {0, 0, 0, 0, 0, 0, 0, 0, 0, 0};
@@ -763,6 +832,19 @@
 #else
 #define GQ_LAP(i) { }
 #endif
+        if (p.vals_out) {
+            for (int32_t r0 = 64 * (int32_t)wv; r0 < size; r0 += 64 * WAVES) {
+                const int32_t ps = r0 + (int32_t)lane;
+                const bool in = ps < size;
+                const uint32_t key = in ? kmer_key(kmer_words(p.residues, wi.aa_off + (uint32_t)ps), s_lut) : KH_NO_KEY;
+                BucketLoads bl;
+                probe_issue<false>(p.table, 1u, p.n_buckets, p.nontemporal != 0u, key, 0u, bl);
+                uint32_t extra = 0;
+                const uint32_t v = probe_finish(p.table, 1u, p.n_buckets, p.nontemporal != 0u, bl, key, extra);
+                if (in) p.vals_out[wi.aa_off + (uint32_t)ps] = v;
+            }
+            __syncthreads();
+        }
         pc.clear();
         for (int32_t r0 = 0; r0 < size; r0 += 64 * WAVES * NWIN)
             count_windows<NullTable, NWIN, true>(p, vals, size, r0 + 64 * (int32_t)wv, 64 * WAVES, nt, pc, s_pref[wv]);
@@ -1279,6 +1361,7 @@
     int g_grid, p_grid, n_cu, pack_grid, pack_grid_long;
     bool use_group;
     bool count_async;
+    bool fused_probe;
     int unit_windows;
     uint32_t pack_shift;
     kaamer_query_meta *d_q;
@@ -1380,16 +1463,21 @@
     return KAAMER_OK;
 }
 
-static void launch_group(const CountParams &p, int grid, bool firstpos, hipStream_t s, bool async, int unit_windows)
-{
+static void launch_group(const CountParams &p, int grid, bool firstpos, hipStream_t s, bool async, int unit_windows, bool fused)
+{
+    if (fused) {
+        if (firstpos) hipLaunchKernelGGL((count_async_kernel<true, true>), dim3(grid), dim3(64 * GRP_WAVES), 0, s, p);
+        else hipLaunchKernelGGL((count_async_kernel<false, true>), dim3(grid), dim3(64 * GRP_WAVES), 0, s, p);
+        return;
+    }
     if (!async && unit_windows == 4) {
         if (firstpos) hipLaunchKernelGGL((count_group_kernel<true, 0, 4>), dim3(grid), dim3(64 * GRP_WAVES), 0, s, p);
         else hipLaunchKernelGGL((count_group_kernel<false, 0, 4>), dim3(grid), dim3(64 * GRP_WAVES), 0, s, p);
         return;
     }
     if (async) {
-        if (firstpos) hipLaunchKernelGGL((count_async_kernel<true>), dim3(grid), dim3(64 * GRP_WAVES), 0, s, p);
-        else hipLaunchKernelGGL((count_async_kernel<false>), dim3(grid), dim3(64 * GRP_WAVES), 0, s, p);
+        if (firstpos) hipLaunchKernelGGL((count_async_kernel<true, false>), dim3(grid), dim3(64 * GRP_WAVES), 0, s, p);
+        else hipLaunchKernelGGL((count_async_kernel<false, false>), dim3(grid), dim3(64 * GRP_WAVES), 0, s, p);
         return;
     }
     if (firstpos) hipLaunchKernelGGL((count_group_kernel<true, 0>), dim3(grid), dim3(64 * GRP_WAVES), 0, s, p);
@@ -1612,11 +1700,18 @@
     }
     ws->firstpos = opts->first_pos == 1 || (opts->first_pos == 0 && (opts->seq_type == KAAMER_NUCLEOTIDE || opts->seq_type == KAAMER_READS));
     int grp_per_cu = 0, p_per_cu = 0;
-    ws->count_async = false;
+    const bool fused_ok = !ws->nucleotide && opts->want_positions == 0;
+    ws->fused_probe = fused_ok && opts->concurrent_batches <= 1 && !getenv("KAAMER_COUNT_ASYNC") && !getenv("KAAMER_COUNT_GROUP") &&
+                      !getenv("KAAMER_COUNT_PACK");
+    if (const char *e = getenv("KAAMER_FUSED_PROBE")) ws->fused_probe = fused_ok && atoi(e) != 0;
+    ws->count_async = ws->fused_probe;
     if (const char *e = getenv("KAAMER_COUNT_ASYNC")) ws->count_async = atoi(e) != 0;
-    hipError_t oe = ws->count_async
-        ? (ws->firstpos ? hipOccupancyMaxActiveBlocksPerMultiprocessor(&grp_per_cu, count_async_kernel<true>, 64 * GRP_WAVES, 0)
-                        : hipOccupancyMaxActiveBlocksPerMultiprocessor(&grp_per_cu, count_async_kernel<false>, 64 * GRP_WAVES, 0))
+    hipError_t oe = ws->fused_probe
+        ? (ws->firstpos ? hipOccupancyMaxActiveBlocksPerMultiprocessor(&grp_per_cu, count_async_kernel<true, true>, 64 * GRP_WAVES, 0)
+                        : hipOccupancyMaxActiveBlocksPerMultiprocessor(&grp_per_cu, count_async_kernel<false, true>, 64 * GRP_WAVES, 0))
+        : ws->count_async
+        ? (ws->firstpos ? hipOccupancyMaxActiveBlocksPerMultiprocessor(&grp_per_cu, count_async_kernel<true, false>, 64 * GRP_WAVES, 0)
+                        : hipOccupancyMaxActiveBlocksPerMultiprocessor(&grp_per_cu, count_async_kernel<false, false>, 64 * GRP_WAVES, 0))
         : (ws->firstpos ? hipOccupancyMaxActiveBlocksPerMultiprocessor(&grp_per_cu, count_group_kernel<true, 0>, 64 * GRP_WAVES, 0)
                         : hipOccupancyMaxActiveBlocksPerMultiprocessor(&grp_per_cu, count_group_kernel<false, 0>, 64 * GRP_WAVES, 0));
     if (oe == hipSuccess)
@@ -1888,6 +1983,7 @@
     uint32_t *status = ws->d_list_counts + SLOT_STATUS;
     uint32_t *queue_head = ws->d_list_counts + SLOT_QUEUE_HEAD;
     const int pb = 256;
+    const bool fused = ws->fused_probe && !nucl && ix->hdr.n_shards <= 1;
     const uint8_t *residues = d_seqs;
     uint64_t pos_bound = seq_bytes;
     uint32_t nq_bound = n_seqs;
@@ -1909,6 +2005,7 @@
         pl.d_total = ws->d_lay_total;
         pl.slot_scale = ws->d_slot_scale;
         pl.room_slots = ws->table_room;
+        pl.no_bitmap = fused ? 1u : 0u;
         const uint32_t tiles = (uint32_t)(((uint64_t)n_seqs + 1 + PL_TILE - 1) / PL_TILE);
         hipLaunchKernelGGL(prep_layout_schedule_kernel, dim3(tiles), dim3(LAY_THREADS), 0, s, pl);
     } else {
@@ -1992,7 +2089,7 @@
     if (p_blocks < 1) p_blocks = 1;
     if (timed) HIPCHK(hipEventRecord(ev[1], s));
     if (ws->nucleotide) hipLaunchKernelGGL(probe_kernel<true>, dim3((unsigned)p_blocks), dim3(64 * P_WAVES), 0, s, pp);
-    else hipLaunchKernelGGL(probe_kernel<false>, dim3((unsigned)p_blocks), dim3(64 * P_WAVES), 0, s, pp);
+    else if (!fused) hipLaunchKernelGGL(probe_kernel<false>, dim3((unsigned)p_blocks), dim3(64 * P_WAVES), 0, s, pp);
     if (timed) HIPCHK(hipEventRecord(ev[2], s));
     const bool split = ws->count_stream && ws->count_stream != s && !timed;
     if (split) {
@@ -2004,6 +2101,12 @@
     memset(&p, 0, sizeof p);
     p.arena = ix->d_arena;
     p.vals = ws->d_vals;
+    if (fused) {
+        p.table = pp.table;
+        p.n_buckets = pp.n_buckets;
+        p.residues = residues;
+        p.nontemporal = pp.nontemporal;
+    }
     p.qinfo = ws->d_qinfo;
     p.slot_off = ws->d_slot_off;
     p.group_first = ws->d_group_first;
@@ -2040,7 +2143,7 @@
         if (ws->use_group) {
             uint64_t gg = ((uint64_t)GRP_MIN_TABLE * nq_bound + 3 * pos_bound) / GRP_BUDGET + 1;
             if (gg > (uint64_t)ws->grp_grid) gg = ws->grp_grid;
-            launch_group(pc, (int)gg, ws->firstpos, s, ws->count_async, ws->unit_windows);
+            launch_group(pc, (int)gg, ws->firstpos, s, ws->count_async, ws->unit_windows, fused);
         } else if (ws->nucleotide) {
             const bool long_orfs = seq_bytes > 200ull * (n_seqs ? n_seqs : 1u) || ws->dense_tables;
             uint64_t g2 = gb;
@@ -2056,6 +2159,7 @@
     }
     CountParams pg = p;
     pg.list = list_ptr(LIST_G); pg.list_count = ws->d_list_counts + LIST_G;
+    if (fused) pg.vals_out = ws->d_vals;
     int g_grid = ws->g_grid;
     if ((uint32_t)g_grid > nq_bound) g_grid = nq_bound > 0 ? (int)nq_bound : 1;
     const bool fused_finalize = !ws->compact && !ws->want_positions;
```
